# Geunwoo-Jeon/LarvaNet

Measured on AMD Instinct MI355X. Metric: HR Mpixels/s (LarvaNet x4 multi-exit train step, 48x48 LR patches), higher is better.
Workload: dtype f32; 1 GPU; LarvaNet x4 train_step_larva M4 B4,4,4,4 48ch, batch 16 of 3x48x48 -> 3x192x192 fp32 per GPU (BASELINE config 2); global_batch=16, parallelism=dp1, hip_graph=True

## Files before the change

### larvanet_amd/build.py

```python
import os
import shutil
import subprocess
import sys

CSRC = os.path.join(os.path.dirname(os.path.abspath(__file__)), "csrc")
LIB = os.path.join(CSRC, "liblarva_hip.so")
SOURCES = ["conv3x3_mfma.hip", "wgrad3x3_mfma.hip", "larva_pointwise.hip", "larva_scale.hip", "conv3x3_f16.hip",
           "larva_metrics.hip", "larva_ensemble.hip", "larva_downscale.hip", "larva_yuv.hip", "larva_resize.hip"]
HEADERS = ["larva_common.h", "larva_bicubic.h", "larva_loss.h"]
FLAGS = ["--offload-arch=gfx950", "-O3", "-std=c++17", "-fPIC", "-Wall", "-Wno-unused-function"]


def _hipcc():
    exe = shutil.which("hipcc") or "/opt/rocm/bin/hipcc"
    if not os.path.exists(exe):
        raise RuntimeError("hipcc not found: the larvanet_amd HIP library cannot be built")
    return exe


def _check_ring_waits(temps, verbose):
    import glob
    asm = glob.glob(os.path.join(temps, "conv3x3_mfma-hip-amdgcn-*.s"))
    obj = os.path.join(temps, "conv3x3_mfma.o")
    if not asm or not os.path.exists(obj):
        raise RuntimeError("larvanet_amd.build: no device assembly from the conv kernel's compile (-save-temps)")
    checker = os.path.join(os.path.dirname(os.path.dirname(CSRC)), "tools", "check_aux_loads.py")
    r = subprocess.run([sys.executable, checker, asm[0]], stdout=subprocess.PIPE, stderr=subprocess.STDOUT)
    tail = r.stdout.decode(errors="replace").strip().splitlines()[-1:]
    if verbose:
        print("[larvanet_amd.build] ring waits vs emitted loads (tools/check_aux_loads.py):", " ".join(tail), flush=True)
    if r.returncode != 0:
        sys.stderr.write(r.stdout.decode(errors="replace"))
        raise RuntimeError("larvanet_amd.build: a counted vmcnt wait of conv3x3_mfma.hip does not match the loads hipcc emitted")
    os.replace(obj, os.path.join(CSRC, "conv3x3_mfma.o"))


def _stale(target, deps):
    if not os.path.exists(target):
        return True
    t = os.path.getmtime(target)
    return any(os.path.getmtime(d) > t for d in deps)


def build_extension(force=False, verbose=True):
    import tempfile
    hipcc = _hipcc()
    hdrs = [os.path.join(CSRC, h) for h in HEADERS]
    objs = []
    procs = []
    temps = None
    for src in SOURCES:
        s = os.path.join(CSRC, src)
        o = os.path.join(CSRC, src.replace(".hip", ".o"))
        objs.append(o)
        if force or _stale(o, [s] + hdrs):
            cmd = [hipcc] + FLAGS + ["-c", s, "-o", o]
            if src == "conv3x3_mfma.hip":
                temps = tempfile.mkdtemp(prefix="build_", dir=CSRC)
                cmd = [hipcc] + FLAGS + ["-save-temps=obj", "-c", s, "-o", os.path.join(temps, "conv3x3_mfma.o")]
            if verbose:
                print("[larvanet_amd.build]", " ".join(cmd), flush=True)
            procs.append((cmd, subprocess.Popen(cmd, stdout=subprocess.PIPE, stderr=subprocess.STDOUT)))
    try:
        for cmd, p in procs:
            out, _ = p.communicate()
            if p.returncode != 0:
                sys.stderr.write(out.decode(errors="replace"))
                raise RuntimeError("hipcc failed: " + " ".join(cmd))
        if temps is not None:
            _check_ring_waits(temps, verbose)
    finally:
        if temps is not None:
            shutil.rmtree(temps, ignore_errors=True)
    if force or procs or _stale(LIB, objs):
        cmd = [hipcc, "--offload-arch=gfx950", "-shared", "-fPIC", "-o", LIB] + objs
        if verbose:
            print("[larvanet_amd.build]", " ".join(cmd), flush=True)
        subprocess.run(cmd, check=True)
    return LIB


if __name__ == "__main__":
    build_extension(force="--force" in sys.argv)
    print(LIB)
```

### larvanet_amd/csrc/conv3x3_mfma.hip

```cpp
#include "larva_common.h"
#include "larva_bicubic.h"
#include <hip/hip_ext.h>
#include <cstdlib>
#include <type_traits>

#ifndef LARVA_DIAG
#define LARVA_DIAG 0
#endif
constexpr int kWgPerCu = 2;
constexpr int kOperandDepth = 2;


#ifndef LARVA_DIAG_ONLY48
#define LARVA_DIAG_ONLY48 0
#endif

namespace larva {

#if defined(LARVA_DIAG) && (LARVA_DIAG & 32)
__device__ unsigned long long* g_stamps = nullptr;
#if LARVA_DIAG & 512
constexpr int kDiagWgPerSlot = 256;
__device__ int g_slot_of_launch = 0;
__device__ __forceinline__ void stamp_slot(unsigned long long* area, int k) {
  if (!area || threadIdx.x != 0 || blockIdx.x >= kDiagWgPerSlot) return;
  const int idx = k == 0 ? 0 : k == 2 ? 1 : k == 3 ? 2 : k == 5 ? 3
                  : !(LARVA_DIAG & 2048) ? -1 : k == 6 ? 5 : k == 7 ? 6 : k == 14 ? 7 : k == 15 ? 8 : k == 1 ? 9 : -1;
  if (idx < 0) return;
  unsigned long long* p = area + (size_t)blockIdx.x * 16;
  p[idx] = __builtin_amdgcn_s_memrealtime();
  if (k == 0) {
    const unsigned hw = __builtin_amdgcn_s_getreg((31 << 11) | 4);
    const unsigned xcc = __builtin_amdgcn_s_getreg((31 << 11) | 20);
    p[4] = (unsigned long long)hw | ((unsigned long long)xcc << 32);
  }
}
#define stamp(k) stamp_slot(a.diag_area, (k))
#else
__device__ __forceinline__ void stamp(int k) {
  if (g_stamps && threadIdx.x == 0)
    g_stamps[blockIdx.x * 16 + k] = (LARVA_DIAG & 64) ? __builtin_amdgcn_s_memtime() : __builtin_amdgcn_s_memrealtime();
}
#endif
#else
__device__ __forceinline__ void stamp(int) {}
#endif

constexpr int kCh = 8;

template <int ROWS_, int COLS_>
struct TileGeo {
  static constexpr int ROWS = ROWS_, COLS = COLS_;
  static constexpr int HALO = ROWS + 2;
  static constexpr int PC = COLS / 16;
  static constexpr int RS = COLS + 8;
  static constexpr int PS = ((HALO * RS + 15) / 32) * 32 + 16;
  static_assert(COLS % 16 == 0 && PS >= HALO * RS && PS % 32 == 16, "tile geometry");
};
using GeoWide = TileGeo<kTileRows, kTileCols>;
using GeoWide4 = TileGeo<4, kTileCols>;
using GeoS5 = TileGeo<5, 16>;
using GeoS4 = TileGeo<4, 16>;
static_assert(GeoWide::RS == kRS && GeoWide::PS == 304, "the 3 x 48 tile of larva_common.h");

struct ConvArgs {
  const float* src[kMaxSrc];
  const float* wpk;
  const float* bias;
  const float* res0;
  const float* res1;
  const float* mask;
  const float* base;
  float* out;
  int cin_per_src;
  int n_chunks;
  int N, H, W;
  int pitch;
  int tiles_x, tiles_y;
  int nwg;
  const unsigned* tile_tab;
  const float* truth;
  float* grad;
  float* partial;
  int plain_stores;
  int tab_n;
  alignas(64) int tab16[32];
  float gval;
  unsigned long long magic_tx, magic_ty, magic_cps;
#if LARVA_DIAG & 512
  unsigned long long* diag_area;
#endif
};

__host__ __device__ __forceinline__ unsigned long long div_magic(int d) { return ((1ull << 40) + d - 1) / (unsigned)d; }
__device__ __forceinline__ int div_by_magic(int n, unsigned long long magic) {
  return (int)(((unsigned long long)(unsigned)n * magic) >> 40);
}

enum Epi : int {
  kEpiPlain = 0,
  kEpiRelu = 1,
  kEpiMask = 2,
  kEpiRes1 = 3,
  kEpiRes2 = 4,
  kEpiShuffle = 5,
  kEpiShuffleBase = 6,
  kEpiShuffleL1 = 7,
  kEpiCount = 8
};

template <int COUT, typename G = GeoWide>
struct ConvCfg {
  static constexpr int CT = COUT / 16;
  static constexpr int CS = cout_stride(COUT);
  static constexpr int PS = G::PS;
  static constexpr int IN_PIECES = (kCh * PS + 255) / 256;
  static constexpr int IN_FLOATS = IN_PIECES * 256;
  static constexpr int IN_SLOTS_PER_PLANE = PS / 4;
  static constexpr int W_USED = 9 * kCh * CS;
  static constexpr int W_PIECES = (W_USED + 255) / 256;
  static constexpr int W_FLOATS = W_PIECES * 256;
  static constexpr int PIECES = IN_PIECES + W_PIECES;
  static constexpr int NPW = (PIECES + 3) / 4;
  static constexpr int STAGE_FLOATS = IN_FLOATS + W_FLOATS;
  static constexpr int STEPS = 9 * (kCh / 4);
  static constexpr int NST = 3;
  static constexpr int AHEAD = NST - 1;
  static constexpr size_t LDS_BYTES_DMA = NST * STAGE_FLOATS * sizeof(float);
  static constexpr bool LOADER = 2 * PIECES <= 63;
  static constexpr int THREADS_DMA = LOADER ? 320 : 256;
  static constexpr size_t LDS_BYTES_REG = 2 * STAGE_FLOATS * sizeof(float);
  static constexpr int RIN_SLOTS = kCh * G::HALO * (G::RS / 4);
  static constexpr int RIN_ITERS = (RIN_SLOTS + 255) / 256;
  static constexpr int RW_SLOTS = W_USED / 4;
  static constexpr int RW_ITERS = (RW_SLOTS + 255) / 256;
  static_assert(kCh * PS <= IN_FLOATS, "input planes must fit their pieces");
};

template <int COUT, typename G>
struct DmaPlan {
  unsigned voff[ConvCfg<COUT, G>::NPW];
};

template <int COUT, typename G, bool WEIGHTS>
__device__ __forceinline__ void make_plan(const ConvArgs& a, int wave, int lane, int y0, int x0,
                                          DmaPlan<COUT, G>& pl) {
  using C = ConvCfg<COUT, G>;
#pragma unroll
  for (int i = 0; i < C::NPW; ++i) {
    const int p = min(wave + 4 * i, C::PIECES - 1);
    const bool isw = p >= C::IN_PIECES;
    if constexpr (WEIGHTS) {
      if (4 * i + 3 < C::IN_PIECES) continue;
      const int ws = (p - C::IN_PIECES) * 64 + lane;
      if (isw) pl.voff[i] = (ws * 4 < C::W_USED) ? 16u * (unsigned)ws : kDmaZero;
    } else {
      if (4 * i >= C::IN_PIECES) continue;
      const int slot = p * 64 + lane;
      const int ci = slot / C::IN_SLOTS_PER_PLANE;
      const int rem = slot - ci * C::IN_SLOTS_PER_PLANE;
      const int r = rem / (G::RS / 4);
      const int q = rem - r * (G::RS / 4);
      const int gy = y0 - 1 + r, gx = x0 - 4 + 4 * q;
      const bool ok = ci < kCh && r < G::HALO && gy >= 0 && gy < a.H && gx >= 0 && gx < a.W;
      if (!isw) pl.voff[i] = ok ? 4u * (unsigned)((ci * a.H + gy) * a.pitch + gx) : kDmaZero;
    }
  }
}

struct ChunkSrc {
  i32x4 img;
  i32x4 wgt;
  const float* img_ptr;
  const float* wgt_ptr;
};

template <int COUT, typename G>
__device__ __forceinline__ ChunkSrc chunk_src(const ConvArgs& a, int chunk, int n, const float* src_override = nullptr) {
  using C = ConvCfg<COUT, G>;
  const int c0 = chunk * kCh;
  const int s_idx = div_by_magic(chunk, a.magic_cps);
  const int c_in_src = c0 - s_idx * a.cin_per_src;
  ChunkSrc cs;
  const float* src = src_override ? src_override : a.src[0];
  if (s_idx != 0) {
    asm volatile("" ::: "memory");
    src = a.src[s_idx];
  }
  cs.img_ptr = src + ((size_t)n * a.cin_per_src + c_in_src) * ((size_t)a.H * a.pitch);
  cs.wgt_ptr = a.wpk + (size_t)chunk * C::W_USED;
  cs.img = dma_rsrc(cs.img_ptr);
  cs.wgt = dma_rsrc(cs.wgt_ptr);
  return cs;
}

template <int COUT, typename G>
__device__ __forceinline__ void dma_piece(const DmaPlan<COUT, G>& pl, int i, int wave, const ChunkSrc& cs,
                                          unsigned stage_addr) {
  using C = ConvCfg<COUT, G>;
  const int p = min(wave + 4 * i, C::PIECES - 1);
  const bool isw = p >= C::IN_PIECES;
  i32x4 rsrc;
#pragma unroll
  for (int k = 0; k < 4; ++k) rsrc[k] = isw ? cs.wgt[k] : cs.img[k];
  lds_dma16_buf(rsrc, pl.voff[i], 0, stage_addr + 1024u * (unsigned)p);
}

template <int COUT, typename G>
struct LoaderPlan {
  unsigned voff[ConvCfg<COUT, G>::PIECES];
};

template <int COUT, typename G>
__device__ __forceinline__ void make_loader_plan(const ConvArgs& a, int lane, int y0, int x0, LoaderPlan<COUT, G>& pl) {
  using C = ConvCfg<COUT, G>;
#pragma unroll
  for (int p = 0; p < C::PIECES; ++p) {
    if (p < C::IN_PIECES) {
      const int slot = p * 64 + lane;
      const int ci = slot / C::IN_SLOTS_PER_PLANE;
      const int rem = slot - ci * C::IN_SLOTS_PER_PLANE;
      const int r = rem / (G::RS / 4);
      const int q = rem - r * (G::RS / 4);
      const int gy = y0 - 1 + r, gx = x0 - 4 + 4 * q;
      const bool ok = ci < kCh && r < G::HALO && gy >= 0 && gy < a.H && gx >= 0 && gx < a.W;
      pl.voff[p] = ok ? 4u * (unsigned)((ci * a.H + gy) * a.pitch + gx) : kDmaZero;
    } else {
      const int ws = (p - C::IN_PIECES) * 64 + lane;
      pl.voff[p] = (ws * 4 < C::W_USED) ? 16u * (unsigned)ws : kDmaZero;
    }
  }
}

template <int COUT, typename G>
__device__ __forceinline__ void run_loader(const ConvArgs& a, float* smem, int lane, int n, int y0, int x0) {
  using C = ConvCfg<COUT, G>;
  if constexpr ((LARVA_DIAG & 256) != 0) return;
  LoaderPlan<COUT, G> pl;
  make_loader_plan<COUT, G>(a, lane, y0, x0, pl);
  const int last = a.n_chunks - 1;
  int stage = 0;
  for (int chunk = 0; chunk <= last; ++chunk) {
    asm volatile("; LARVA_RING loader chunk_pieces=%1 ahead=%2\n\ts_waitcnt vmcnt(%0)\n\ts_barrier" ::"n"((C::AHEAD - 1) * C::PIECES), "n"(C::PIECES), "n"(C::AHEAD) : "memory");
    __builtin_amdgcn_sched_barrier(0);
    const int nstage = (stage + C::AHEAD) % C::NST;
    const unsigned dst = lds_addr_of(smem + nstage * C::STAGE_FLOATS);
    const ChunkSrc cs = chunk_src<COUT, G>(a, min(chunk + C::AHEAD, last), n);
#pragma unroll
    for (int p = 0; p < C::PIECES; ++p)
      lds_dma16_buf(p < C::IN_PIECES ? cs.img : cs.wgt, pl.voff[p], 0, dst + 1024u * (unsigned)p);
    stage = stage == C::NST - 1 ? 0 : stage + 1;
  }
  asm volatile("s_waitcnt vmcnt(0)" ::: "memory");
}

template <int COUT, typename G>
struct RegStaging {
  f32x4 in[ConvCfg<COUT, G>::RIN_ITERS];
  f32x4 w[ConvCfg<COUT, G>::RW_ITERS];
};

template <int COUT, typename G>
__device__ __forceinline__ void reg_load(const ConvArgs& a, const ChunkSrc& cs, int y0, int x0, int tid,
                                         RegStaging<COUT, G>& st) {
  using C = ConvCfg<COUT, G>;
  const size_t plane = (size_t)a.H * a.pitch;
#pragma unroll
  for (int i = 0; i < C::RIN_ITERS; ++i) {
    const int s = min(tid + i * 256, C::RIN_SLOTS - 1);
    const int ci = s / (G::HALO * (G::RS / 4));
    const int rem = s - ci * (G::HALO * (G::RS / 4));
    const int r = rem / (G::RS / 4);
    const int q = rem - r * (G::RS / 4);
    const int gy = y0 - 1 + r, gx = x0 - 4 + 4 * q;
    const bool row_ok = gy >= 0 && gy < a.H;
    const float* row = cs.img_ptr + (size_t)ci * plane + (size_t)min(max(gy, 0), a.H - 1) * a.pitch;
    f32x4 v;
#pragma unroll
    for (int e = 0; e < 4; ++e) {
      const int x = gx + e;
      const float t = row[min(max(x, 0), a.W - 1)];
      v[e] = (row_ok && x >= 0 && x < a.W) ? t : 0.f;
    }
    st.in[i] = v;
  }
#pragma unroll
  for (int i = 0; i < C::RW_ITERS; ++i) {
    const int s = min(tid + i * 256, C::RW_SLOTS - 1);
    const float* p = cs.wgt_ptr + 4 * s;
    st.w[i] = f32x4{p[0], p[1], p[2], p[3]};
  }
}

template <int COUT, typename G>
__device__ __forceinline__ void reg_store(float* stage, int tid, const RegStaging<COUT, G>& st) {
  using C = ConvCfg<COUT, G>;
#pragma unroll
  for (int i = 0; i < C::RIN_ITERS; ++i) {
    const int s = tid + i * 256;
    if (s < C::RIN_SLOTS) {
      const int ci = s / (G::HALO * (G::RS / 4));
      const int rem = s - ci * (G::HALO * (G::RS / 4));
      const int r = rem / (G::RS / 4);
      const int q = rem - r * (G::RS / 4);
      *reinterpret_cast<f32x4*>(stage + ci * C::PS + r * G::RS + 4 * q) = st.in[i];
    }
  }
#pragma unroll
  for (int i = 0; i < C::RW_ITERS; ++i) {
    const int s = tid + i * 256;
    if (s < C::RW_SLOTS) *reinterpret_cast<f32x4*>(stage + C::IN_FLOATS + 4 * s) = st.w[i];
  }
}

template <int COUT, typename G, int NCT, int PG0, int NPG>
__device__ __forceinline__ void read_operands(const float* const (&a_base)[NCT], const float* b_base, int step,
                                              float (&av)[NCT], float (&bv)[NPG]) {
  using C = ConvCfg<COUT, G>;
  if constexpr ((LARVA_DIAG & 128) != 0) {
#pragma unroll
    for (int c = 0; c < NCT; ++c) av[c] = (float)step;
#pragma unroll
    for (int p = 0; p < NPG; ++p) bv[p] = (float)(step + p);
    return;
  }
  const int tap = step / (kCh / 4), kk = step % (kCh / 4);
  const int ky = tap / 3, kx = tap % 3;
#pragma unroll
  for (int c = 0; c < NCT; ++c) av[c] = a_base[c][(tap * kCh + kk * 4) * C::CS];
#pragma unroll
  for (int p = 0; p < NPG; ++p) {
    const int pg = PG0 + p, prow = pg / G::PC, pcol = pg % G::PC;
    bv[p] = b_base[kk * 4 * C::PS + (prow + ky) * G::RS + pcol * 16 + kx];
  }
}

template <int NMF, int NRD, int M>
__device__ __forceinline__ void shadow_groups() {
  if constexpr (M < NMF) {
    __builtin_amdgcn_sched_group_barrier(0x8, 1, 0);
    constexpr int share = (NRD + NMF - 1 - M) / NMF;
    if constexpr (share > 0) __builtin_amdgcn_sched_group_barrier(0x100, share, 0);
    shadow_groups<NMF, NRD, M + 1>();
  }
}

template <int COUT, typename G, int NCT, int PG0, int NPG, bool SWAP>
__device__ __forceinline__ void mfma_chunk(const float* stage, int ct0, int lane, f32x4 (&acc)[NCT][NPG],
                                           const float* wstage = nullptr) {
  using C = ConvCfg<COUT, G>;
  const int lr = lane & 15, lq = lane >> 4;
  const float* const wrows = wstage ? wstage : stage + C::IN_FLOATS;
  const float* a_base[NCT];
#pragma unroll
  for (int c = 0; c < NCT; ++c)
    a_base[c] = wrows + lq * C::CS + lr + (cout_swizzled(COUT) ? (((ct0 + c) ^ (lq & 1)) * 16) : (ct0 + c) * 16);
  const float* b_base = stage + lq * C::PS + lr + 3;
  constexpr int D = kOperandDepth;
  float av[D + 1][NCT], bv[D + 1][NPG];
#pragma unroll
  for (int d = 0; d < D; ++d)
    if (d < C::STEPS) read_operands<COUT, G, NCT, PG0, NPG>(a_base, b_base, d, av[d], bv[d]);
#pragma unroll
  for (int step = 0; step < C::STEPS; ++step) {
    __builtin_amdgcn_sched_barrier(0);
    if (step + D < C::STEPS)
      read_operands<COUT, G, NCT, PG0, NPG>(a_base, b_base, step + D, av[(step + D) % (D + 1)], bv[(step + D) % (D + 1)]);
    constexpr int NMF = NCT * NPG;
    constexpr int NRD = NCT + NPG;
#pragma unroll
    for (int m = 0; m < NMF; ++m) {
      const float wv = av[step % (D + 1)][m / NPG], xv = bv[step % (D + 1)][m % NPG];
      acc[m / NPG][m % NPG] = __builtin_amdgcn_mfma_f32_16x16x4f32(SWAP ? xv : wv, SWAP ? wv : xv, acc[m / NPG][m % NPG], 0, 0, 0);
    }
    shadow_groups<NMF, NRD, 0>();
    __builtin_amdgcn_sched_barrier(0);
  }
}

template <int KEEP, int PIECES, int AUX>
__device__ __forceinline__ void wait_and_barrier() {
  static_assert(KEEP == PIECES + AUX, "a ring wait keeps exactly the next chunk's pieces and the operand loads in flight");
  asm volatile("; LARVA_RING pieces=%1 aux=%2\n\ts_waitcnt vmcnt(%0)\n\ts_barrier" ::"n"(KEEP), "n"(PIECES), "n"(AUX) : "memory");
  __builtin_amdgcn_sched_barrier(0);
}

template <typename G>
__device__ __forceinline__ void decode_tile(const ConvArgs& a, int vb, int& n, int& y0, int& x0) {
  const int tile = xcd_remap(vb, a.nwg);
  const int t2 = div_by_magic(tile, a.magic_tx);
  const int tx = tile - t2 * a.tiles_x;
  n = div_by_magic(t2, a.magic_ty);
  const int ty = t2 - n * a.tiles_y;
  x0 = tx * G::COLS;
  y0 = ty * G::ROWS;
}

template <int COUT, typename G, bool VEC, int EPI, int NCT, int PG0, int NPG, bool PERSIST = false>
__device__ __forceinline__ void run_role(const ConvArgs& a, float* smem, int ct0, int wave, int n, int y0, int x0, int tid) {
  using C = ConvCfg<COUT, G>;
  static_assert(!VEC || C::LOADER, "the 16-byte path runs with a loader wave (2 * PIECES <= 63 for every instantiated shape)");
  static_assert(!PERSIST || VEC, "persistent tiles: the loader-wave path");
  const int lane = tid & 63;
  const int lr = lane & 15, lq = lane >> 4;
  float* const out_ptr = a.out;
  struct { int H, W, pitch, plain; } k = {a.H, a.W, a.pitch, a.plain_stores};
  asm volatile("" : "+s"(k.H), "+s"(k.W), "+s"(k.pitch), "+s"(k.plain));

  constexpr bool kShuffleEpi = (EPI == kEpiShuffle || EPI == kEpiShuffleBase || EPI == kEpiShuffleL1);
  constexpr bool kPixMajor = VEC && !kShuffleEpi;
  f32x4 bias[NCT];
#pragma unroll
  for (int c = 0; c < NCT; ++c) bias[c] = f32x4{0.f, 0.f, 0.f, 0.f};
  auto load_bias = [&]() {
    if (a.bias) {
#pragma unroll
      for (int c = 0; c < NCT; ++c)
#pragma unroll
        for (int r = 0; r < 4; ++r) bias[c][r] = a.bias[(ct0 + c) * 16 + (kPixMajor ? lr : lq * 4 + r)];
    }
  };

  constexpr int NAUX = (EPI == kEpiMask || EPI == kEpiRes1 || EPI == kEpiShuffleBase)
                           ? 1 : ((EPI == kEpiRes2 || EPI == kEpiShuffleL1) ? 2 : 0);
  f32x4 aux[NAUX > 0 ? NAUX : 1][NAUX > 0 ? NCT : 1][NAUX > 0 ? NPG : 1];
  constexpr int NU = NCT * NPG;
  constexpr int kEarlyPairs = PERSIST && COUT == 48 ? (NAUX * NU < 7 ? NAUX * NU : 7) : NAUX * NU;
  constexpr int kLatePart = 4, kEarlyAll = 5;
  auto load_aux = [&](int part = -1) {
#pragma unroll
    for (int c = 0; c < NCT; ++c)
#pragma unroll
      for (int p = 0; p < NPG; ++p) {
        const int pg = PG0 + p, prow = pg / G::PC, pcol = pg % G::PC;
        const int y = min(y0 + prow, a.H - 1), x = min(x0 + pcol * 16 + lr, a.W - 1);
        auto want = [&](int op) {
          const int q = op * NU + c * NPG + p;
          return part < 0 ? true : part == kLatePart ? q >= kEarlyPairs : q < kEarlyPairs;
        };
        if constexpr (kShuffleEpi) {
          const int HH = 4 * a.H, WW = 4 * a.W;
          const size_t idx = (((size_t)n * C::CT + (ct0 + c)) * HH + (4 * y + lq)) * WW + 4 * x;
          if (want(0)) aux[0][c][p] = *reinterpret_cast<const f32x4*>(a.base + idx);
          if constexpr (EPI == kEpiShuffleL1) {
            if (want(1)) aux[1][c][p] = *reinterpret_cast<const f32x4*>(a.truth + idx);
          }
        } else if constexpr (kPixMajor && (PERSIST || G::COLS == 16)) {
          const unsigned plane = (unsigned)a.H * (unsigned)a.pitch;
          const unsigned lane_off = 4u * ((unsigned)lr * plane + (unsigned)lq * 4u);
          const int soff = __builtin_amdgcn_readfirstlane(
              (int)(4u * ((unsigned)((ct0 + c) * 16) * plane + (unsigned)(y0 + prow) * (unsigned)a.pitch + (unsigned)(x0 + pcol * 16))));
          auto image = [&](const float* t) {
            const unsigned long long b = reinterpret_cast<unsigned long long>(t + (size_t)n * COUT * plane);
            const unsigned lo = (unsigned)__builtin_amdgcn_readfirstlane((int)(unsigned)b);
            const unsigned hi = (unsigned)__builtin_amdgcn_readfirstlane((int)(unsigned)(b >> 32));
            return __builtin_amdgcn_make_buffer_rsrc(reinterpret_cast<void*>(((unsigned long long)hi << 32) | lo), 0,
                                                     (int)(COUT * plane * 4u), 0x00020000);
          };
          if constexpr (EPI == kEpiMask) {
            if (want(0)) aux[0][c][p] = __builtin_bit_cast(f32x4, __builtin_amdgcn_raw_buffer_load_b128(image(a.mask), lane_off, soff, 0));
          }
          if constexpr (EPI == kEpiRes1 || EPI == kEpiRes2) {
            if (want(0)) aux[0][c][p] = __builtin_bit_cast(f32x4, __builtin_amdgcn_raw_buffer_load_b128(image(a.res0), lane_off, soff, 0));
          }
          if constexpr (EPI == kEpiRes2) {
            if (want(1)) aux[1][c][p] = __builtin_bit_cast(f32x4, __builtin_amdgcn_raw_buffer_load_b128(image(a.res1), lane_off, soff, 0));
          }
        } else if constexpr (kPixMajor) {
          const size_t plane = (size_t)a.H * a.pitch;
          const int xb = min(x0 + pcol * 16 + lq * 4, a.pitch - 4);
          const size_t idx = ((size_t)n * COUT + (ct0 + c) * 16 + lr) * plane + (size_t)y * a.pitch + xb;
          if constexpr (EPI == kEpiMask) {
            if (want(0)) aux[0][c][p] = *reinterpret_cast<const f32x4*>(a.mask + idx);
          }
          if constexpr (EPI == kEpiRes1 || EPI == kEpiRes2) {
            if (want(0)) aux[0][c][p] = *reinterpret_cast<const f32x4*>(a.res0 + idx);
          }
          if constexpr (EPI == kEpiRes2) {
            if (want(1)) aux[1][c][p] = *reinterpret_cast<const f32x4*>(a.res1 + idx);
          }
        } else {
          const size_t plane = (size_t)a.H * a.pitch;
          const size_t idx0 = ((size_t)n * COUT + (ct0 + c) * 16 + lq * 4) * plane + (size_t)y * a.pitch + x;
#pragma unroll
          for (int r = 0; r < 4; ++r) {
            if constexpr (EPI == kEpiMask) aux[0][c][p][r] = a.mask[idx0 + r * plane];
            if constexpr (EPI == kEpiRes1 || EPI == kEpiRes2) aux[0][c][p][r] = a.res0[idx0 + r * plane];
            if constexpr (EPI == kEpiRes2) aux[1][c][p][r] = a.res1[idx0 + r * plane];
          }
        }
      }
  };
  constexpr bool kAuxLate = VEC && !kShuffleEpi && !(LARVA_DIAG & 6) && NAUX > 0 && !PERSIST;
  constexpr int kAuxLoads = kAuxLate ? NAUX * NCT * NPG : 0;
  auto load_early = [&]() {
    load_bias();
    if constexpr (NAUX > 0 && !kAuxLate && !(LARVA_DIAG & 4)) load_aux();
  };
  int pstage = 0;
  for (int vb = blockIdx.x;; vb += gridDim.x) {
  if constexpr (PERSIST) {
    if (vb >= a.nwg) break;
    decode_tile<G>(a, vb, n, y0, x0);
  }
  if constexpr (!VEC || (LARVA_DIAG & 2)) load_early();

  f32x4 acc[NCT][NPG];
#pragma unroll
  for (int c = 0; c < NCT; ++c)
#pragma unroll
    for (int p = 0; p < NPG; ++p) acc[c][p] = f32x4{0.f, 0.f, 0.f, 0.f};

  if constexpr (PERSIST) {
    load_bias();
    const int my_chunk = a.n_chunks >= 4 ? (wave & 3) : 0;
    __builtin_amdgcn_sched_barrier(0);
    for (int chunk = 0; chunk < a.n_chunks; ++chunk) {
      asm volatile("s_barrier" ::: "memory");
      __builtin_amdgcn_sched_barrier(0);
      if constexpr (NAUX > 0) {
        if (chunk == my_chunk) load_aux(kEarlyAll);
        __builtin_amdgcn_sched_barrier(0);
      }
      mfma_chunk<COUT, G, NCT, PG0, NPG, kPixMajor>(smem + pstage * C::STAGE_FLOATS, ct0, lane, acc);
      pstage = pstage == C::NST - 1 ? 0 : pstage + 1;
    }
    asm volatile("s_waitcnt vmcnt(0)" ::: "memory");
    __builtin_amdgcn_sched_barrier(0);
    if constexpr (kEarlyPairs < NAUX * NU) {
      load_aux(kLatePart);
      __builtin_amdgcn_sched_barrier(0);
    }
  } else if constexpr (VEC) {
    DmaPlan<COUT, G> pl;
    const int last = a.n_chunks - 1;
    if constexpr (!(LARVA_DIAG & 2)) {
      const ChunkSrc cs0 = chunk_src<COUT, G>(a, 0, n);
      const unsigned st0 = lds_addr_of(smem), st1 = lds_addr_of(smem + C::STAGE_FLOATS);
      stamp(6);
      make_plan<COUT, G, true>(a, wave, lane, y0, x0, pl);
#pragma unroll
      for (int i = 0; i < C::NPW; ++i)
        if (wave + 4 * i >= C::IN_PIECES) dma_piece<COUT, G>(pl, i, wave, cs0, st0);
      __builtin_amdgcn_sched_barrier(0);
      stamp(7);
      load_early();
      stamp(14);
      make_plan<COUT, G, false>(a, wave, lane, y0, x0, pl);
#pragma unroll
      for (int i = 0; i < C::NPW; ++i)
        if (wave + 4 * i < C::IN_PIECES) dma_piece<COUT, G>(pl, i, wave, cs0, st0);
      stamp(15);
      const ChunkSrc cs1 = chunk_src<COUT, G>(a, min(1, last), n);
#pragma unroll
      for (int i = 0; i < C::NPW; ++i) dma_piece<COUT, G>(pl, i, wave, cs1, st1);
      if constexpr (kAuxLate) {
        __builtin_amdgcn_sched_barrier(0);
        load_aux();
        __builtin_amdgcn_sched_barrier(0);
      }
    }
    stamp(1);
    int stage = 0;
    for (int chunk = 0; chunk <= last; ++chunk) {
      if constexpr ((LARVA_DIAG & 256) != 0) {
      } else if (chunk == 0) wait_and_barrier<((LARVA_DIAG & 2) ? 0 : C::NPW) + kAuxLoads, ((LARVA_DIAG & 2) ? 0 : C::NPW), kAuxLoads>();
      else wait_and_barrier<kAuxLoads, 0, kAuxLoads>();
      if (chunk == 0) stamp(2);
      stamp(8 + (chunk < 7 ? chunk : 7));
      if constexpr (!(LARVA_DIAG & 1)) mfma_chunk<COUT, G, NCT, PG0, NPG, kPixMajor>(smem + stage * C::STAGE_FLOATS, ct0, lane, acc);
      stage = stage == C::NST - 1 ? 0 : stage + 1;
    }
    asm volatile("s_waitcnt vmcnt(0)" ::: "memory");
    stamp(3);
  } else {
    RegStaging<COUT, G> st;
    if constexpr (!(LARVA_DIAG & 2)) {
      reg_load<COUT, G>(a, chunk_src<COUT, G>(a, 0, n), y0, x0, tid, st);
      reg_store<COUT, G>(smem, tid, st);
    }
    __syncthreads();
    for (int chunk = 0; chunk < a.n_chunks; ++chunk) {
      float* cur = smem + (chunk & 1) * C::STAGE_FLOATS;
      float* nxt = smem + ((chunk & 1) ^ 1) * C::STAGE_FLOATS;
      const bool more = chunk + 1 < a.n_chunks;
      if constexpr (!(LARVA_DIAG & 2)) {
        if (more) reg_load<COUT, G>(a, chunk_src<COUT, G>(a, chunk + 1, n), y0, x0, tid, st);
      }
      if constexpr (!(LARVA_DIAG & 1)) mfma_chunk<COUT, G, NCT, PG0, NPG, kPixMajor>(cur, ct0, lane, acc);
      if constexpr (!(LARVA_DIAG & 2)) {
        if (more) reg_store<COUT, G>(nxt, tid, st);
      }
      __syncthreads();
    }
  }

  if constexpr ((LARVA_DIAG & 4) != 0) {
#pragma unroll
    for (int c = 0; c < NCT; ++c)
#pragma unroll
      for (int p = 0; p < NPG; ++p) asm volatile("" ::"v"(acc[c][p]));
    return;
  }

  if constexpr (EPI == kEpiShuffleL1) {
    const int HH = 4 * k.H, WW = 4 * k.W;
    const size_t plane = (size_t)k.H * k.pitch;
    const float g = a.gval;
    float s = 0.f;
#pragma unroll
    for (int c = 0; c < NCT; ++c)
#pragma unroll
      for (int p = 0; p < NPG; ++p) {
        const int pg = PG0 + p, prow = pg / G::PC, pcol = pg % G::PC;
        const int y = y0 + prow, x = x0 + pcol * 16 + lr;
        const f32x4 v = (acc[c][p] + bias[c]) + aux[0][c][p];
        if (y < k.H && x < k.W) {
          if (out_ptr) {
            const size_t idx = (((size_t)n * C::CT + (ct0 + c)) * HH + (4 * y + lq)) * WW + 4 * x;
            __builtin_nontemporal_store(v, reinterpret_cast<f32x4*>(out_ptr + idx));
          }
          const f32x4 d = v - aux[1][c][p];
          s += fabsf(d[0]) + fabsf(d[1]) + fabsf(d[2]) + fabsf(d[3]);
          const size_t idx0 = ((size_t)n * COUT + (ct0 + c) * 16 + lq * 4) * plane + (size_t)y * k.pitch + x;
#pragma unroll
          for (int r = 0; r < 4; ++r)
            __builtin_nontemporal_store(d[r] > 0.f ? g : (d[r] < 0.f ? -g : 0.f), &a.grad[idx0 + r * plane]);
        }
      }
#pragma unroll
    for (int o = 32; o > 0; o >>= 1) s += __shfl_xor(s, o);
    if (lane == 0) a.partial[4 * blockIdx.x + wave] = s;
  } else if constexpr (EPI == kEpiShuffle || EPI == kEpiShuffleBase) {
    const int HH = 4 * k.H, WW = 4 * k.W;
#pragma unroll
    for (int c = 0; c < NCT; ++c)
#pragma unroll
      for (int p = 0; p < NPG; ++p) {
        const int pg = PG0 + p, prow = pg / G::PC, pcol = pg % G::PC;
        const int y = y0 + prow, x = x0 + pcol * 16 + lr;
        const size_t idx = (((size_t)n * C::CT + (ct0 + c)) * HH + (4 * y + lq)) * WW + 4 * x;
        f32x4 v = acc[c][p] + bias[c];
        if constexpr (EPI == kEpiShuffleBase) v += aux[0][c][p];
        if (y < k.H && x < k.W) __builtin_nontemporal_store(v, reinterpret_cast<f32x4*>(out_ptr + idx));
      }
  } else if constexpr (kPixMajor) {
    const size_t plane = (size_t)k.H * k.pitch;
    auto store_all = [&](auto plain_tag, auto interior_tag) {
      constexpr bool kPlain = decltype(plain_tag)::value;
      constexpr bool kInterior = decltype(interior_tag)::value;
#pragma unroll
      for (int c = 0; c < NCT; ++c)
#pragma unroll
        for (int p = 0; p < NPG; ++p) {
          const int pg = PG0 + p, prow = pg / G::PC, pcol = pg % G::PC;
          const int y = y0 + prow, xb = x0 + pcol * 16 + lq * 4;
          const size_t idx = ((size_t)n * COUT + (ct0 + c) * 16 + lr) * plane + (size_t)y * k.pitch + xb;
          f32x4 v = acc[c][p] + bias[c];
          if (kInterior || (y < k.H && xb < k.pitch)) {
#pragma unroll
            for (int r = 0; r < 4; ++r) {
              float o = v[r];
              if constexpr (EPI == kEpiRelu) o = fmaxf(o, 0.f);
              if constexpr (EPI == kEpiMask) o = (aux[0][c][p][r] > 0.f) ? o : 0.f;
              if constexpr (EPI == kEpiRes1 || EPI == kEpiRes2) o += aux[0][c][p][r];
              if constexpr (EPI == kEpiRes2) o += aux[1][c][p][r];
              v[r] = (kInterior || xb + r < k.W) ? o : 0.f;
            }
            if constexpr (kPlain) *reinterpret_cast<f32x4*>(out_ptr + idx) = v;
            else __builtin_nontemporal_store(v, reinterpret_cast<f32x4*>(out_ptr + idx));
          }
        }
    };
    constexpr bool kFastPath = EPI == kEpiPlain || EPI == kEpiRelu || EPI == kEpiRes1;
    const bool interior = kFastPath && y0 + G::ROWS <= k.H && x0 + G::COLS <= k.W;
    auto store_policy = [&](auto plain_tag) {
      if constexpr (kFastPath) {
        if (interior) {
          store_all(plain_tag, std::true_type{});
          return;
        }
      }
      store_all(plain_tag, std::false_type{});
    };
    if constexpr ((LARVA_DIAG & 16) != 0) {
      store_policy(std::true_type{});
    } else if constexpr (G::COLS == 16) {
      if (k.plain) store_policy(std::true_type{});
      else store_policy(std::false_type{});
    } else {
      store_policy(std::false_type{});
    }
  } else {
    const size_t plane = (size_t)k.H * k.pitch;
#pragma unroll
    for (int c = 0; c < NCT; ++c)
#pragma unroll
      for (int p = 0; p < NPG; ++p) {
        const int pg = PG0 + p, prow = pg / G::PC, pcol = pg % G::PC;
        const int y = y0 + prow, x = x0 + pcol * 16 + lr;
        const size_t idx0 = ((size_t)n * COUT + (ct0 + c) * 16 + lq * 4) * plane + (size_t)y * k.pitch + x;
        const f32x4 v = acc[c][p] + bias[c];
        if (y < k.H && x < k.pitch) {
          const bool real = x < k.W;
#pragma unroll
          for (int r = 0; r < 4; ++r) {
            float o = v[r];
            if constexpr (EPI == kEpiRelu) o = fmaxf(o, 0.f);
            if constexpr (EPI == kEpiMask) o = (aux[0][c][p][r] > 0.f) ? o : 0.f;
            if constexpr (EPI == kEpiRes1 || EPI == kEpiRes2) o += aux[0][c][p][r];
            if constexpr (EPI == kEpiRes2) o += aux[1][c][p][r];
            o = real ? o : 0.f;
            if constexpr ((LARVA_DIAG & 16) != 0) out_ptr[idx0 + r * plane] = o;
            else __builtin_nontemporal_store(o, &out_ptr[idx0 + r * plane]);
          }
        }
      }
  }
#if LARVA_DIAG & 32
  stamp(4);
  asm volatile("s_waitcnt vmcnt(0)" ::: "memory");
  stamp(5);
#endif
  if constexpr (!PERSIST) break;
  }
}

__device__ __forceinline__ void fetch_args(const ConvArgs& a) {
  asm volatile("" ::"s"(a.src[0]), "s"(a.wpk), "s"(a.bias), "s"(a.out), "s"(a.cin_per_src), "s"(a.n_chunks), "s"(a.N),
               "s"(a.H), "s"(a.W), "s"(a.pitch), "s"(a.tiles_x), "s"(a.tiles_y), "s"(a.magic_tx), "s"(a.magic_ty),
               "s"(a.magic_cps), "s"(a.nwg), "s"(a.tile_tab), "s"(a.plain_stores), "s"(a.tab_n),
               "s"(a.tab16[0]), "s"(a.tab16[16]));
}

template <int COUT, bool VEC, int EPI, typename G = GeoWide>
__device__ __forceinline__ void conv_tile(const ConvArgs& a, float* smem) {
  if constexpr ((LARVA_DIAG & 8) != 0) return;
  stamp(0);
  fetch_args(a);
  const int tile = xcd_remap(blockIdx.x, a.nwg);
  const int t2 = div_by_magic(tile, a.magic_tx);
  const int tx = tile - t2 * a.tiles_x;
  const int n = div_by_magic(t2, a.magic_ty);
  const int ty = t2 - n * a.tiles_y;
  const int x0 = tx * G::COLS, y0 = ty * G::ROWS;
  const int tid = threadIdx.x;
  const int wave = __builtin_amdgcn_readfirstlane(tid >> 6);
  __builtin_amdgcn_s_setprio(1);

  if constexpr (VEC) {
    if (wave == 4) {
      if constexpr (!(LARVA_DIAG & 2)) run_loader<COUT, G>(a, smem, tid & 63, n, y0, x0);
      return;
    }
  }
  if constexpr (G::ROWS == 4) {
    static_assert(VEC && (COUT == 48 || COUT == 32), "4 x 48 tiles: the 16-byte path at 48 / 32 channels");
    if constexpr (COUT == 48) {
      if (wave < 3) run_role<COUT, G, VEC, EPI, 1, 0, 9>(a, smem, wave, wave, n, y0, x0, tid);
      else run_role<COUT, G, VEC, EPI, 3, 9, 3>(a, smem, 0, wave, n, y0, x0, tid);
    } else {
      if (wave < 2) run_role<COUT, G, VEC, EPI, 1, 0, 6>(a, smem, wave, wave, n, y0, x0, tid);
      else run_role<COUT, G, VEC, EPI, 1, 6, 6>(a, smem, wave - 2, wave, n, y0, x0, tid);
    }
  } else if constexpr (COUT == 48) {
    if (wave < 3) run_role<COUT, G, VEC, EPI, 1, 0, 7>(a, smem, wave, wave, n, y0, x0, tid);
    else run_role<COUT, G, VEC, EPI, 3, 7, 2>(a, smem, 0, wave, n, y0, x0, tid);
  } else if constexpr (COUT == 32) {
    if (wave < 2) run_role<COUT, G, VEC, EPI, 1, 0, 5>(a, smem, wave, wave, n, y0, x0, tid);
    else run_role<COUT, G, VEC, EPI, 1, 5, 4>(a, smem, wave - 2, wave, n, y0, x0, tid);
  } else {
    static_assert(COUT == 64, "unsupported channel count");
    run_role<COUT, G, VEC, EPI, 1, 0, 9>(a, smem, wave, wave, n, y0, x0, tid);
  }
}

template <int COUT, bool VEC, int EPI>
__global__ __launch_bounds__(VEC ? ConvCfg<COUT>::THREADS_DMA : 256, VEC ? kWgPerCu : 1) void conv3x3_mfma_kernel(ConvArgs a) {
  extern __shared__ __attribute__((aligned(16))) float smem[];
  conv_tile<COUT, VEC, EPI>(a, smem);
}

template <int COUT, int EPI>
__global__ __launch_bounds__((ConvCfg<COUT, GeoWide4>::THREADS_DMA), kWgPerCu) void conv3x3_mfma_rows4_kernel(ConvArgs a) {
  extern __shared__ __attribute__((aligned(16))) float smem[];
  conv_tile<COUT, true, EPI, GeoWide4>(a, smem);
}
static_assert(2 * ConvCfg<48, GeoWide4>::LDS_BYTES_DMA <= 160 * 1024, "two 4 x 48 workgroups per CU");

template <int COUT, typename G>
__device__ __forceinline__ void run_loader_persist(const ConvArgs& a, float* smem, int lane) {
  using C = ConvCfg<COUT, G>;
  static_assert(C::NST == 3 && 2 * C::PIECES <= 63, "three stages, two chunks in flight");
  LoaderPlan<COUT, G> pl;
  int vb_i = blockIdx.x, n_i, y0, x0, c_i = 0, s_i = 0;
  decode_tile<G>(a, vb_i, n_i, y0, x0);
  make_loader_plan<COUT, G>(a, lane, y0, x0, pl);
  bool more = true;
  auto issue = [&]() {
    const ChunkSrc cs = chunk_src<COUT, G>(a, c_i, n_i);
    const unsigned dst = lds_addr_of(smem + s_i * C::STAGE_FLOATS);
#pragma unroll
    for (int p = 0; p < C::PIECES; ++p)
      lds_dma16_buf(p < C::IN_PIECES ? cs.img : cs.wgt, pl.voff[p], 0, dst + 1024u * (unsigned)p);
    s_i = s_i == C::NST - 1 ? 0 : s_i + 1;
    if (++c_i == a.n_chunks) {
      c_i = 0;
      vb_i += gridDim.x;
      more = vb_i < a.nwg;
      if (more) {
        decode_tile<G>(a, vb_i, n_i, y0, x0);
        make_loader_plan<COUT, G>(a, lane, y0, x0, pl);
      }
    }
  };
  int ahead = 0;
  issue();
  ++ahead;
  if (more) {
    issue();
    ++ahead;
  }
  while (ahead > 0) {
    if (ahead == 2) asm volatile("s_waitcnt vmcnt(%0)" ::"n"(C::PIECES) : "memory");
    else asm volatile("s_waitcnt vmcnt(0)" ::: "memory");
    asm volatile("s_barrier" ::: "memory");
    __builtin_amdgcn_sched_barrier(0);
    --ahead;
    if (more) {
      issue();
      ++ahead;
    }
  }
}

template <int COUT, int EPI>
__global__ __launch_bounds__((ConvCfg<COUT>::THREADS_DMA), kWgPerCu) void conv3x3_mfma_persist_kernel(ConvArgs a) {
  extern __shared__ __attribute__((aligned(16))) float smem[];
  using G = GeoWide;
  stamp(0);
  fetch_args(a);
  const int tid = threadIdx.x;
  const int wave = __builtin_amdgcn_readfirstlane(tid >> 6);
  __builtin_amdgcn_s_setprio(1);
  if (wave == 4) {
    run_loader_persist<COUT, G>(a, smem, tid & 63);
    return;
  }
  if constexpr (COUT == 48) {
    if (wave < 3) run_role<COUT, G, true, EPI, 1, 0, 7, true>(a, smem, wave, wave, 0, 0, 0, tid);
    else run_role<COUT, G, true, EPI, 3, 7, 2, true>(a, smem, 0, wave, 0, 0, 0, tid);
  } else if constexpr (COUT == 32) {
    if (wave < 2) run_role<COUT, G, true, EPI, 1, 0, 5, true>(a, smem, wave, wave, 0, 0, 0, tid);
    else run_role<COUT, G, true, EPI, 1, 5, 4, true>(a, smem, wave - 2, wave, 0, 0, 0, tid);
  } else {
    static_assert(COUT == 64, "unsupported channel count");
    run_role<COUT, G, true, EPI, 1, 0, 9, true>(a, smem, wave, wave, 0, 0, 0, tid);
  }
}

template <int COUT, int EPI, typename G>
__device__ __forceinline__ void strip_roles(const ConvArgs& a, float* smem, int wave, int n, int y0, int x0, int tid) {
  static_assert(ConvCfg<COUT, G>::LOADER, "the strip kernel is launched with a loader wave");
  static_assert(COUT == 48 || COUT == 32 || COUT == 64, "strip tiles: 32, 48 or 64 output channels");
  if (wave == 4) {
    run_loader<COUT, G>(a, smem, tid & 63, n, y0, x0);
    return;
  }
  if constexpr (COUT == 64) {
    run_role<COUT, G, true, EPI, 1, 0, G::ROWS>(a, smem, wave, wave, n, y0, x0, tid);
  } else if constexpr (COUT == 48) {
    if (wave < 3) run_role<COUT, G, true, EPI, 1, 0, G::ROWS - 1>(a, smem, wave, wave, n, y0, x0, tid);
    else run_role<COUT, G, true, EPI, 3, G::ROWS - 1, 1>(a, smem, 0, wave, n, y0, x0, tid);
  } else if constexpr (G::ROWS == 5) {
    if (wave < 2) run_role<COUT, G, true, EPI, 1, 0, 3>(a, smem, wave, wave, n, y0, x0, tid);
    else if (wave == 2) run_role<COUT, G, true, EPI, 2, 3, 1>(a, smem, 0, wave, n, y0, x0, tid);
    else run_role<COUT, G, true, EPI, 2, 4, 1>(a, smem, 0, wave, n, y0, x0, tid);
  } else {
    if (wave < 2) run_role<COUT, G, true, EPI, 1, 0, 2>(a, smem, wave, wave, n, y0, x0, tid);
    else run_role<COUT, G, true, EPI, 1, 2, 2>(a, smem, wave - 2, wave, n, y0, x0, tid);
  }
}

template <int COUT, int EPI>
__global__ __launch_bounds__(320, kWgPerCu) void conv3x3_mfma_strip_kernel(ConvArgs a) {
  extern __shared__ __attribute__((aligned(16))) float smem[];
  stamp(0);
  fetch_args(a);
  const int tile = xcd_remap(blockIdx.x, a.nwg);
  const int n = div_by_magic(tile, a.magic_tx);
  const int slot = tile - n * a.tiles_x;
  unsigned e;
  if (a.tab_n) {
    const unsigned pair = (unsigned)a.tab16[slot >> 1];
    const unsigned h = (slot & 1) ? pair >> 16 : pair & 0xffffu;
    e = (h & 0xffu) | (((h >> 8) & 0x7fu) << 16) | ((h >> 15) << 31);
  } else {
    e = a.tile_tab[slot];
  }
  const int y0 = (int)(e & 0xfffu), x0 = (int)((e >> 12) & 0xfffu);
  const int tid = threadIdx.x;
  const int wave = __builtin_amdgcn_readfirstlane(tid >> 6);
  __builtin_amdgcn_s_setprio(1);
  if (e >> 31) strip_roles<COUT, EPI, GeoS5>(a, smem, wave, n, y0, x0, tid);
  else strip_roles<COUT, EPI, GeoS4>(a, smem, wave, n, y0, x0, tid);
}
template <int COUT>
constexpr size_t kStripLdsBytes = ConvCfg<COUT, GeoS5>::LDS_BYTES_DMA > ConvCfg<COUT, GeoS4>::LDS_BYTES_DMA ? ConvCfg<COUT, GeoS5>::LDS_BYTES_DMA
                                                                                                            : ConvCfg<COUT, GeoS4>::LDS_BYTES_DMA;
static_assert(kWgPerCu * kStripLdsBytes<48> <= 160 * 1024 && kWgPerCu * kStripLdsBytes<64> <= 160 * 1024, "strip workgroups per CU");

constexpr int kMaxConvJobs = 4;
struct ConvBatch {
  ConvArgs job[kMaxConvJobs];
};

template <int COUT, int EPI>
__global__ __launch_bounds__(ConvCfg<COUT>::THREADS_DMA, kWgPerCu) void conv3x3_mfma_batch_kernel(ConvBatch b) {
  extern __shared__ __attribute__((aligned(16))) float smem[];
  conv_tile<COUT, true, EPI>(b.job[blockIdx.y], smem);
}

constexpr int kMaxPackJobs = 64;

struct PackJob {
  const float* w;
  float* fwd;
  float* bwd;
  int cout, cin, w_cin_total, w_cin_off;
};

struct PackBatch {
  PackJob job[kMaxPackJobs];
};

__host__ __device__ constexpr int packed_floats(int cout, int cin) {
  return (cin / kCh) * 9 * kCh * cout_stride(cout);
}

constexpr int kPackTileCols = 64;
constexpr int kPackLd = kPackTileCols + 1;
constexpr int kPackTileFloats = 9 * kCh * kPackLd;

__host__ __device__ constexpr int pack_slots(int cout, int cin) { return cin / kCh + cout / kCh; }

__device__ __forceinline__ void pack_block(const PackJob& j, int slot, float* __restrict__ tile) {
  const int nfc = j.cin / kCh;
  const bool fwd = slot < nfc;
  const int chunk = fwd ? slot : slot - nfc;
  float* __restrict__ out = fwd ? j.fwd : j.bwd;
  if ((!fwd && chunk >= j.cout / kCh) || !out) return;
  const int cols = fwd ? j.cout : j.cin;
  const int cs = cout_stride(cols);
  const int tid = threadIdx.x;
  out += (size_t)chunk * 72 * cs;
  for (int c0 = 0; c0 < cs; c0 += kPackTileCols) {
    const int ncol = min(kPackTileCols, cols - c0);
    if (fwd) {
      for (int idx = tid; idx < ncol * 72; idx += 256) {
        const int c = idx / 72, r = idx - c * 72, k = r / 9, tap = r - k * 9;
        const int cin_abs = j.w_cin_off + chunk * kCh + k;
        tile[(tap * kCh + k) * kPackLd + c] =
            cin_abs < j.w_cin_total ? j.w[((size_t)(c0 + c) * j.w_cin_total + cin_abs) * 9 + tap] : 0.f;
      }
    } else {
      const int row = ncol * 9;
      for (int idx = tid; idx < kCh * row; idx += 256) {
        const int k = idx / row, rem = idx - k * row, c = rem / 9, tap = rem - c * 9;
        tile[((8 - tap) * kCh + k) * kPackLd + c] =
            j.w_cin_off + c0 + c < j.w_cin_total
                ? j.w[((size_t)(chunk * kCh + k) * j.w_cin_total + j.w_cin_off + c0) * 9 + rem] : 0.f;
      }
    }
    __syncthreads();
    const int wcols = min(kPackTileCols, cs - c0);
    const bool swz = cout_swizzled(cols);
    for (int idx = tid; idx < 72 * wcols; idx += 256) {
      const int r = idx / wcols, c = idx - r * wcols;
      const int col = swz ? ((c0 + c) ^ ((r & 1) << 4)) : c0 + c;
      out[r * cs + col] = c < ncol ? tile[r * kPackLd + c] : 0.f;
    }
    __syncthreads();
  }
}

__global__ __launch_bounds__(256) void pack_weights_batch_kernel(PackBatch b) {
  __shared__ float tile[kPackTileFloats];
  pack_block(b.job[blockIdx.y], blockIdx.x, tile);
}

constexpr int kPrologueBlocks = 192;
constexpr int kProloguePadSlices = 2, kPrologueBicSlices = 8;
struct PrologueArgs {
  PackBatch packs;
  int npack, slots;
  const float* x;
  float* x16;
  float* base;
  int N, C, H, W;
};

__global__ __launch_bounds__(256) void step_prologue_kernel(PrologueArgs a) {
  __shared__ float tile[kPackTileFloats];
  int blk = blockIdx.x;
  if (blk < a.npack * a.slots) {
    const int job = blk / a.slots;
    pack_block(a.packs.job[job], blk - job * a.slots, tile);
    return;
  }
  blk -= a.npack * a.slots;
  constexpr int nthr = kPrologueBlocks * 256;
  const int slice = blk / kPrologueBlocks, tid = (blk - slice * kPrologueBlocks) * 256 + threadIdx.x;
  const int nbic = a.base ? kPrologueBicSlices : 0;
  if (slice < nbic) {
    bicubic4_body(a.x, a.base, a.N * a.C, a.H, a.W, (long long)slice * nthr + tid, (long long)nthr * kPrologueBicSlices);
  } else {
    const int plane = a.H * a.W, per_img = a.C * plane, total = a.N * per_img;
    for (int i = (slice - nbic) * nthr + tid; i < total; i += nthr * kProloguePadSlices) {
      const int n = i / per_img, r = i - n * per_img;
      a.x16[(size_t)n * 16 * plane + r] = a.x[i];
    }
  }
}

struct LaunchTiming {
  hipEvent_t start, stop;
};

template <auto Kernel, typename Args>
static hipError_t launch(dim3 grid, dim3 block, size_t lds, hipStream_t stream, const LaunchTiming* tm, const Args& a) {
  static PerDeviceOnce lds_set;
  if (const hipError_t e = ensure_dynamic_lds(lds_set, reinterpret_cast<const void*>(Kernel), lds); e != hipSuccess) return e;
  if (tm)
    hipExtLaunchKernelGGL(Kernel, grid, block, lds, stream, tm->start, tm->stop, 0, a);
  else
    hipLaunchKernelGGL(Kernel, grid, block, lds, stream, a);
  return hipGetLastError();
}

template <int... E>
struct EpiSet {
  static constexpr bool has(int epi) { return ((epi == E) || ...); }
};
using EpiAll = EpiSet<kEpiPlain, kEpiRelu, kEpiMask, kEpiRes1, kEpiRes2, kEpiShuffle, kEpiShuffleBase>;
using EpiBatch48 = EpiSet<kEpiPlain, kEpiRelu, kEpiMask, kEpiRes1, kEpiRes2, kEpiShuffle, kEpiShuffleBase, kEpiShuffleL1>;
using EpiInference = EpiSet<kEpiPlain, kEpiRelu, kEpiRes1, kEpiRes2, kEpiShuffle, kEpiShuffleBase>;
using EpiRows4 = EpiInference;
using EpiPersist = EpiInference;

template <int... E, typename F>
static hipError_t with_epi(EpiSet<E...>, int epi, hipError_t absent, F&& f) {
  hipError_t r = absent;
  (void)((epi == E && (r = f(std::integral_constant<int, E>{}), true)) || ...);
  return r;
}

template <typename F>
static hipError_t with_cout(int cout, hipError_t absent, F&& f) {
  switch (cout) {
#if !LARVA_DIAG_ONLY48
    case 32: return f(std::integral_constant<int, 32>{});
    case 64: return f(std::integral_constant<int, 64>{});
#endif
    case 48: return f(std::integral_constant<int, 48>{});
    default: return absent;
  }
}

static int conv_slots() { return kWgPerCu * device_cu_count(); }

template <int COUT>
static hipError_t launch_conv(const ConvArgs& a, bool vec, int epi, hipStream_t stream, const LaunchTiming* tm) {
  using C = ConvCfg<COUT>;
  const dim3 grid(a.N * a.tiles_x * a.tiles_y);
  return with_epi(EpiAll{}, epi, hipErrorInvalidValue, [&](auto e) {
    constexpr int EPI = decltype(e)::value;
    if (vec)
      return launch<conv3x3_mfma_kernel<COUT, true, EPI>>(grid, dim3(C::THREADS_DMA), C::LDS_BYTES_DMA, stream, tm, a);
    return launch<conv3x3_mfma_kernel<COUT, false, EPI>>(grid, dim3(256), C::LDS_BYTES_REG, stream, tm, a);
  });
}

template <int COUT>
static hipError_t launch_rows4(const ConvArgs& a, int epi, hipStream_t stream, const LaunchTiming* tm) {
  using C = ConvCfg<COUT, GeoWide4>;
  return with_epi(EpiRows4{}, epi, hipErrorNotSupported, [&](auto e) {
    return launch<conv3x3_mfma_rows4_kernel<COUT, decltype(e)::value>>(dim3(a.nwg), dim3(C::THREADS_DMA), C::LDS_BYTES_DMA,
                                                                      stream, tm, a);
  });
}

template <int COUT>
static hipError_t launch_persist(const ConvArgs& a, int epi, hipStream_t stream, const LaunchTiming* tm) {
  using C = ConvCfg<COUT>;
  if ((long long)COUT * a.H * a.pitch * 4 >= (1ll << 31)) return hipErrorNotSupported;
  const int grid = a.nwg < conv_slots() ? a.nwg : conv_slots();
  return with_epi(EpiPersist{}, epi, hipErrorNotSupported, [&](auto e) {
    return launch<conv3x3_mfma_persist_kernel<COUT, decltype(e)::value>>(dim3(grid), dim3(C::THREADS_DMA), C::LDS_BYTES_DMA,
                                                                        stream, tm, a);
  });
}

template <int COUT>
static hipError_t launch_batch(const ConvBatch& b, int njobs, int epi, hipStream_t stream) {
  using C = ConvCfg<COUT>;
  using Set = std::conditional_t<COUT == 48, EpiBatch48, EpiAll>;
  const ConvArgs& a = b.job[0];
  return with_epi(Set{}, epi, epi == kEpiShuffleL1 ? hipErrorNotSupported : hipErrorInvalidValue, [&](auto e) {
    return launch<conv3x3_mfma_batch_kernel<COUT, decltype(e)::value>>(dim3(a.N * a.tiles_x * a.tiles_y, njobs),
                                                                      dim3(C::THREADS_DMA), C::LDS_BYTES_DMA, stream,
                                                                      nullptr, b);
  });
}

template <int COUT>
static hipError_t launch_strip(const ConvArgs& a, int epi, hipStream_t stream, const LaunchTiming* tm) {
  return with_epi(EpiAll{}, epi, hipErrorInvalidValue, [&](auto e) {
    return launch<conv3x3_mfma_strip_kernel<COUT, decltype(e)::value>>(dim3(a.nwg), dim3(320), kStripLdsBytes<COUT>, stream,
                                                                      tm, a);
  });
}

}

using namespace larva;

extern "C" {

long long larva_packed_weight_floats(int cout, int cin) { return (long long)packed_floats(cout, cin); }

static int fill_pack_jobs(PackBatch& b, const float* const* w, float* const* wpk_fwd, float* const* wpk_bwd,
                          const int* cout, const int* cin, const int* w_cin_total, const int* w_cin_off, int njobs) {
  int slots = 0;
  for (int i = 0; i < njobs; ++i) {
    if (!w[i] || cout[i] % kCh || cin[i] % kCh || cout[i] <= 0 || cin[i] <= 0) return -1;
    b.job[i] = PackJob{w[i], wpk_fwd[i], wpk_bwd[i], cout[i], cin[i], w_cin_total[i], w_cin_off[i]};
    const int n = pack_slots(cout[i], cin[i]);
    slots = n > slots ? n : slots;
  }
  return slots;
}

int larva_pack_weights_batch(const float* const* w, float* const* wpk_fwd, float* const* wpk_bwd,
                             const int* cout, const int* cin, const int* w_cin_total,
                             const int* w_cin_off, int njobs, void* stream) {
  if (njobs < 1 || njobs > kMaxPackJobs) return (int)hipErrorInvalidValue;
  PackBatch b{};
  const int slots = fill_pack_jobs(b, w, wpk_fwd, wpk_bwd, cout, cin, w_cin_total, w_cin_off, njobs);
  if (slots < 1) return (int)hipErrorInvalidValue;
  hipLaunchKernelGGL(pack_weights_batch_kernel, dim3(slots, njobs), dim3(256), 0, (hipStream_t)stream, b);
  return (int)hipGetLastError();
}

int larva_step_prologue(const float* const* w, float* const* wpk_fwd, float* const* wpk_bwd, const int* cout,
                        const int* cin, const int* w_cin_total, const int* w_cin_off, int njobs, const float* x,
                        float* x16, float* base, int N, int C, int H, int W, void* stream) {
  if (njobs < 0 || njobs > kMaxPackJobs || !x || N <= 0 || C <= 0 || C > 16 || H <= 0 || W <= 0)
    return (int)hipErrorInvalidValue;
  if ((long long)N * 16 * H * W >= (1ll << 31)) return (int)hipErrorInvalidValue;
  if (base && (reinterpret_cast<uintptr_t>(base) & 15)) return (int)hipErrorInvalidValue;
  PrologueArgs a{};
  a.slots = njobs ? fill_pack_jobs(a.packs, w, wpk_fwd, wpk_bwd, cout, cin, w_cin_total, w_cin_off, njobs) : 0;
  if (a.slots < 0) return (int)hipErrorInvalidValue;
  a.npack = njobs;
  a.x = x; a.x16 = x16; a.base = base;
  a.N = N; a.C = C; a.H = H; a.W = W;
  if (!x16 && base) return (int)hipErrorInvalidValue;
  const int blocks = njobs * a.slots + kPrologueBlocks * ((base ? kPrologueBicSlices : 0) + (x16 ? kProloguePadSlices : 0));
  if (blocks == 0) return 0;
  hipLaunchKernelGGL(step_prologue_kernel, dim3(blocks), dim3(256), 0, (hipStream_t)stream, a);
  return (int)hipGetLastError();
}

int larva_pack_weights(const float* w, float* wpk_fwd, float* wpk_bwd, int cout, int cin,
                       int w_cin_total, int w_cin_off, void* stream) {
  return larva_pack_weights_batch(&w, &wpk_fwd, &wpk_bwd, &cout, &cin, &w_cin_total, &w_cin_off, 1, stream);
}

#if LARVA_DIAG & 512
static int g_diag_next_slot = -1, g_diag_slot_cap = 0;
static unsigned long long* g_diag_host_base = nullptr;
static int diag_take_slot() {
  if (g_diag_next_slot < 0 || g_diag_next_slot >= g_diag_slot_cap) return -1;
  return g_diag_next_slot++;
}
int larva_diag_arm_slots(int first, int cap) {
  const int was = g_diag_next_slot;
  g_diag_next_slot = first;
  g_diag_slot_cap = cap;
  return was;
}
int larva_diag_next_slot(void) { return g_diag_next_slot; }
#endif

static int conv_build(const float* const* src, int n_src, int cin_per_src, const float* wpk, const float* bias,
                      const float* res0, const float* res1, const float* mask, const float* base, float* out,
                      int N, int H, int W, int pitch, int relu, int mode, ConvArgs& a, bool& aligned, int& epi) {
  if (pitch == 0) pitch = W;
  if (pitch < W) return (int)hipErrorInvalidValue;
  if (n_src < 1 || n_src > kMaxSrc || cin_per_src % kCh || cin_per_src <= 0 || N <= 0 || H <= 0 || W <= 0)
    return (int)hipErrorInvalidValue;
  if (mode != 0 && mode != 1) return (int)hipErrorInvalidValue;
  if ((long long)cin_per_src * H * pitch >= (1ll << 31)) return (int)hipErrorInvalidValue;
  if (!wpk || !out) return (int)hipErrorInvalidValue;
  a = ConvArgs{};
#if LARVA_DIAG & 512
  {
    const int slot = diag_take_slot();
    a.diag_area = (slot >= 0 && g_diag_host_base) ? g_diag_host_base + (size_t)slot * kDiagWgPerSlot * 16 : nullptr;
  }
#endif
  aligned = (pitch % 4 == 0) && ((reinterpret_cast<uintptr_t>(wpk) & 15) == 0);
  for (int i = 0; i < n_src; ++i) {
    if (!src[i]) return (int)hipErrorInvalidValue;
    a.src[i] = src[i];
    aligned = aligned && ((reinterpret_cast<uintptr_t>(src[i]) & 15) == 0);
  }
  aligned = aligned && (((reinterpret_cast<uintptr_t>(out) | reinterpret_cast<uintptr_t>(res0) |
                          reinterpret_cast<uintptr_t>(res1) | reinterpret_cast<uintptr_t>(mask)) & 15) == 0);
  a.wpk = wpk; a.bias = bias; a.res0 = res0; a.res1 = res1; a.mask = mask; a.base = base;
  a.out = out;
  a.cin_per_src = cin_per_src;
  a.n_chunks = n_src * cin_per_src / kCh;
  a.N = N; a.H = H; a.W = W; a.pitch = pitch;
  a.tiles_x = (pitch + kTileCols - 1) / kTileCols;
  a.tiles_y = (H + kTileRows - 1) / kTileRows;
  if ((long long)N * a.tiles_x * a.tiles_y >= (1ll << 20)) return (int)hipErrorInvalidValue;
  a.magic_tx = div_magic(a.tiles_x);
  a.magic_ty = div_magic(a.tiles_y);
  a.magic_cps = div_magic(cin_per_src / kCh);
  a.nwg = N * a.tiles_x * a.tiles_y;
  if (mode == 1) {
    if (relu || mask || res0 || res1) return (int)hipErrorInvalidValue;
    epi = base ? kEpiShuffleBase : kEpiShuffle;
  } else {
    if (base) return (int)hipErrorInvalidValue;
    const int code = (relu ? 1 : 0) | (mask ? 2 : 0) | (res0 ? 4 : 0) | (res1 ? 8 : 0);
    switch (code) {
      case 0: epi = kEpiPlain; break;
      case 1: epi = kEpiRelu; break;
      case 2: epi = kEpiMask; break;
      case 4: epi = kEpiRes1; break;
      case 12: epi = kEpiRes2; break;
      default: return (int)hipErrorInvalidValue;
    }
  }
  return 0;
}

static int conv_tile_rows(int N, int H, int pitch, int cout, int epi, bool aligned, int forced) {
  const bool can4 = aligned && (cout == 48 || cout == 32) && EpiRows4::has(epi);
  if (forced == 3 || !can4) return 3;
  if (forced == 4) return 4;
  const long long tiles3 = (long long)N * ((pitch + kTileCols - 1) / kTileCols) * ((H + 2) / 3);
  return (cout == 32 && tiles3 > conv_slots()) ? 4 : 3;
}

static int conv_dispatch(const float* const* src, int n_src, int cin_per_src, const float* wpk,
                         const float* bias, const float* res0, const float* res1, const float* mask,
                         const float* base, float* out, int N, int cout, int H, int W, int pitch, int relu,
                         int mode, void* stream, const LaunchTiming* tm, int tile_rows = 0) {
  ConvArgs a;
  bool aligned;
  int epi;
  const int rc = conv_build(src, n_src, cin_per_src, wpk, bias, res0, res1, mask, base, out, N, H, W, pitch, relu,
                            mode, a, aligned, epi);
  if (rc) return rc;
  hipStream_t s = (hipStream_t)stream;
  if (tile_rows != 0 && tile_rows != 3 && tile_rows != 4) return (int)hipErrorInvalidValue;
  if (conv_tile_rows(N, H, a.pitch, cout, epi, aligned, tile_rows) == 4) {
    a.tiles_y = (H + 3) / 4;
    a.magic_ty = div_magic(a.tiles_y);
    a.nwg = N * a.tiles_x * a.tiles_y;
    return (int)with_cout(cout, hipErrorInvalidValue, [&](auto c) {
      if constexpr (decltype(c)::value == 64) return hipErrorNotSupported;
      else return launch_rows4<decltype(c)::value>(a, epi, s, tm);
    });
  }
  if (tile_rows == 4) return (int)hipErrorNotSupported;
  const char* pe = getenv("LARVA_PERSIST");
  const bool persist_on = !(pe && pe[0] == '0');
  if (persist_on && aligned && a.nwg > conv_slots()) {
    const hipError_t e = with_cout(cout, hipErrorNotSupported, [&](auto c) {
      return launch_persist<decltype(c)::value>(a, epi, s, tm);
    });
    if (e != hipErrorNotSupported) return (int)e;
  }
  return (int)with_cout(cout, hipErrorInvalidValue, [&](auto c) {
    return launch_conv<decltype(c)::value>(a, aligned, epi, s, tm);
  });
}

int larva_conv3x3_fwd(const float* const* src, int n_src, int cin_per_src, const float* wpk,
                      const float* bias, const float* res0, const float* res1, const float* mask,
                      const float* base, float* out, int N, int cout, int H, int W, int relu,
                      int mode, void* stream) {
  return conv_dispatch(src, n_src, cin_per_src, wpk, bias, res0, res1, mask, base, out, N, cout, H, W, 0, relu,
                       mode, stream, nullptr);
}

int larva_conv3x3_fwd_pitched(const float* const* src, int n_src, int cin_per_src, const float* wpk,
                              const float* bias, const float* res0, const float* res1, const float* mask,
                              const float* base, float* out, int N, int cout, int H, int W, int pitch,
                              int relu, int mode, void* stream) {
  return conv_dispatch(src, n_src, cin_per_src, wpk, bias, res0, res1, mask, base, out, N, cout, H, W, pitch,
                       relu, mode, stream, nullptr);
}

int larva_conv3x3_fwd_tiled(const float* const* src, int n_src, int cin_per_src, const float* wpk,
                            const float* bias, const float* res0, const float* res1, const float* mask,
                            const float* base, float* out, int N, int cout, int H, int W, int pitch,
                            int relu, int mode, int tile_rows, void* stream) {
  return conv_dispatch(src, n_src, cin_per_src, wpk, bias, res0, res1, mask, base, out, N, cout, H, W, pitch,
                       relu, mode, stream, nullptr, tile_rows);
}

int larva_conv3x3_fwd_batch(int njobs, const float* const* src, int n_src, int cin_per_src,
                            const float* const* wpk, const float* const* bias, const float* const* res0,
                            const float* const* res1, const float* const* mask, const float* const* base,
                            float* const* out, int N, int cout, int H, int W, int pitch, int relu, int mode,
                            void* stream) {
  if (njobs < 2 || njobs > kMaxConvJobs || !src || !wpk || !out) return (int)hipErrorInvalidValue;
  ConvBatch b{};
  int epi0 = -1;
  for (int j = 0; j < njobs; ++j) {
    bool aligned;
    int epi;
    const int rc = conv_build(src + (size_t)j * n_src, n_src, cin_per_src, wpk[j], bias ? bias[j] : nullptr,
                              res0 ? res0[j] : nullptr, res1 ? res1[j] : nullptr, mask ? mask[j] : nullptr,
                              base ? base[j] : nullptr, out[j], N, H, W, pitch, relu, mode, b.job[j], aligned, epi);
    if (rc) return rc;
    if (!aligned) return (int)hipErrorNotSupported;
    if (j > 0 && epi != epi0) return (int)hipErrorInvalidValue;
    epi0 = epi;
  }
  return (int)with_cout(cout, hipErrorInvalidValue, [&](auto c) {
    return launch_batch<decltype(c)::value>(b, njobs, epi0, (hipStream_t)stream);
  });
}

int larva_exit_l1_partials(int N, int H, int pitch) {
  return 4 * N * ((pitch + kTileCols - 1) / kTileCols) * ((H + kTileRows - 1) / kTileRows);
}

int larva_conv3x3_exit_l1_batch(int njobs, const float* const* src, int n_src, int cin_per_src,
                                const float* const* wpk, const float* const* bias, const float* const* base,
                                const float* const* truth, float* const* out, float* const* grad,
                                float* const* partial, float gval, int N, int cout, int H, int W, int pitch,
                                void* stream) {
  if (njobs < 2 || njobs > kMaxConvJobs || !src || !wpk || !base || !truth || !out || !grad || !partial)
    return (int)hipErrorInvalidValue;
  if (cout != 48) return (int)hipErrorNotSupported;
  ConvBatch b{};
  for (int j = 0; j < njobs; ++j) {
    bool aligned;
    int epi;
    if (!base[j] || !truth[j] || !grad[j] || !partial[j]) return (int)hipErrorInvalidValue;
    const int rc = conv_build(src + (size_t)j * n_src, n_src, cin_per_src, wpk[j], bias ? bias[j] : nullptr, nullptr,
                              nullptr, nullptr, base[j], grad[j], N, H, W, pitch, 0, 1, b.job[j], aligned, epi);
    if (rc) return rc;
    if (!aligned || ((reinterpret_cast<uintptr_t>(truth[j]) | reinterpret_cast<uintptr_t>(base[j])) & 15))
      return (int)hipErrorNotSupported;
    b.job[j].out = out[j];
    b.job[j].truth = truth[j];
    b.job[j].grad = grad[j];
    b.job[j].partial = partial[j];
    b.job[j].gval = gval;
  }
  return (int)launch_batch<48>(b, njobs, kEpiShuffleL1, (hipStream_t)stream);
}

int larva_strip_tile_table(int H, int W, int phase, unsigned* tab, int cap) {
  if (H <= 0 || W <= 0 || H >= 4096 || W >= 4096 || !tab || cap < 0) return -1;
  int n5 = 0, n4 = 0;
  for (int pass = 0; pass < 2; ++pass) {
    int fives = 0, fours = 0, i5 = 0, i4 = 0;
    for (int x0 = 0; x0 < W; x0 += 16) {
      int best_a = -1, best_gap = 1 << 30;
      for (int a5 = 0; 5 * a5 <= H; ++a5) {
        if ((H - 5 * a5) % 4) continue;
        const int b4 = (H - 5 * a5) / 4;
        const int gap = (fives + a5) - (fours + b4);
        const int g = gap < 0 ? -gap : gap;
        if (g < best_gap) { best_gap = g; best_a = a5; }
      }
      if (best_a < 0) return -2;
      const int a5 = best_a, b4 = (H - 5 * a5) / 4;
      fives += a5; fours += b4;
      if (pass == 0) continue;
      int y = 0, ra = a5, rb = b4;
      while (ra > 0 || rb > 0) {
        const bool five = ra > 0 && (rb == 0 || (long long)ra * b4 >= (long long)rb * a5);
        const int k = five ? i5++ : i4++;
        const int mine = five ? n5 : n4, other = five ? n4 : n5;
        const bool first = five == (phase == 0);
        int slot;
        if (k < other) slot = 2 * k + (first ? 0 : 1);
        else slot = 2 * other + (k - other);
        (void)mine;
        if (slot < cap) tab[slot] = (unsigned)y | ((unsigned)x0 << 12) | (five ? 0x80000000u : 0u);
        y += five ? 5 : 4;
        if (five) --ra; else --rb;
      }
    }
    n5 = fives; n4 = fours;
  }
  return n5 + n4;
}

static int strips_dispatch(const float* const* src, int n_src, int cin_per_src, const float* wpk,
                           const float* bias, const float* res0, const float* res1, const float* mask,
                           const float* base, float* out, int N, int cout, int H, int W, int pitch,
                           int relu, int mode, const unsigned* tile_tab, const unsigned* tile_tab_host,
                           int tiles_per_image, int plain_stores, void* stream, const LaunchTiming* tm) {
  if (cout != 48 && cout != 32 && cout != 64) return (int)hipErrorNotSupported;
  if (!tile_tab || tiles_per_image < 1) return (int)hipErrorInvalidValue;
  ConvArgs a;
  bool aligned;
  int epi;
  const int rc = conv_build(src, n_src, cin_per_src, wpk, bias, res0, res1, mask, base, out, N, H, W, pitch, relu,
                            mode, a, aligned, epi);
  if (rc) return rc;
  if (!aligned) return (int)hipErrorNotSupported;
  if ((long long)N * tiles_per_image >= (1ll << 20)) return (int)hipErrorInvalidValue;
  if ((long long)cout * H * a.pitch * 4 >= (1ll << 31)) return (int)hipErrorNotSupported;
  a.tile_tab = tile_tab;
  if (tile_tab_host && tiles_per_image <= 64 && H <= 256 && pitch <= 2048) {
    a.tab_n = tiles_per_image;
    for (int t = 0; t < tiles_per_image; ++t) {
      const unsigned e = tile_tab_host[t];
      const unsigned y0 = e & 0xfffu, x0 = (e >> 12) & 0xfffu;
      if (y0 > 255u || (x0 & 15u) || (x0 >> 4) > 127u) { a.tab_n = 0; break; }
      const unsigned h = y0 | ((x0 >> 4) << 8) | ((e >> 31) << 15);
      a.tab16[t >> 1] |= (int)(h << ((t & 1) * 16));
    }
  }
  a.plain_stores = plain_stores ? 1 : 0;
  a.tiles_x = tiles_per_image;
  a.tiles_y = 1;
  a.magic_tx = div_magic(tiles_per_image);
  a.magic_ty = div_magic(1);
  a.nwg = N * tiles_per_image;
  return (int)with_cout(cout, hipErrorNotSupported, [&](auto c) {
    return launch_strip<decltype(c)::value>(a, epi, (hipStream_t)stream, tm);
  });
}

int larva_conv3x3_fwd_strips(const float* const* src, int n_src, int cin_per_src, const float* wpk,
                             const float* bias, const float* res0, const float* res1, const float* mask,
                             const float* base, float* out, int N, int cout, int H, int W, int pitch,
                             int relu, int mode, const unsigned* tile_tab, const unsigned* tile_tab_host,
                             int tiles_per_image, int plain_stores, void* stream) {
  return strips_dispatch(src, n_src, cin_per_src, wpk, bias, res0, res1, mask, base, out, N, cout, H, W, pitch, relu, mode,
                         tile_tab, tile_tab_host, tiles_per_image, plain_stores, stream, nullptr);
}

#if LARVA_DIAG & 32
int larva_diag_set_stamps(unsigned long long* buf) {
#if LARVA_DIAG & 512
  g_diag_host_base = buf;
#endif
  return (int)hipMemcpyToSymbol(HIP_SYMBOL(larva::g_stamps), &buf, sizeof(buf));
}
#endif

}
```

Before: 366.0 HR Mpixels/s.

## Preload leading conv kernel arguments into SGPRs and prefetch strip weights early

Conv kernels now take their hot scalar parameters (weight/source pointers, tile magics, sizes) as leading scalar arguments, and the build passes an LLVM flag so that the first kernarg dwords are preloaded into SGPRs. The goal is to remove the kernarg-load latency at the start of each short conv workgroup. The strip kernel also issues the weight DMA before decoding its tile, with WPRE skipping the later weight load and GeoS4 padded to match GeoS5's piece count. A build check enforces that preload is present and that VGPRs stay within 128, which adds build fragility and more register pressure.

Result: slower. 361.9 HR Mpixels/s (-1.1%).

```diff
diff --git a/larvanet_amd/build.py b/larvanet_amd/build.py
--- a/larvanet_amd/build.py
+++ b/larvanet_amd/build.py
@@ -9,6 +9,8 @@
            "larva_metrics.hip", "larva_ensemble.hip", "larva_downscale.hip", "larva_yuv.hip", "larva_resize.hip"]
 HEADERS = ["larva_common.h", "larva_bicubic.h", "larva_loss.h"]
 FLAGS = ["--offload-arch=gfx950", "-O3", "-std=c++17", "-fPIC", "-Wall", "-Wno-unused-function"]
+KERNARG_PRELOAD_DWORDS = 14
+CONV_FLAGS = ["-mllvm", "-amdgpu-kernarg-preload-count=%d" % KERNARG_PRELOAD_DWORDS]
 
 
 def _hipcc():
@@ -35,6 +37,35 @@
     os.replace(obj, os.path.join(CSRC, "conv3x3_mfma.o"))
 
 
+def _check_preload(temps, verbose):
+    import glob
+    import re
+    asm = glob.glob(os.path.join(temps, "conv3x3_mfma-hip-amdgcn-*.s"))
+    text = open(asm[0]).read()
+    kernels = re.findall(r"\.amdhsa_kernel (_ZN5larva\d+conv3x3_mfma_\w*kernel\w+)(.*?)\.end_amdhsa_kernel", text, re.S)
+    if not kernels:
+        raise RuntimeError("larvanet_amd.build: no conv3x3_mfma_*_kernel descriptors in the device assembly")
+
+    def field(body, name):
+        m = re.search(r"\.amdhsa_%s (\d+)" % name, body)
+        return int(m.group(1)) if m else 0
+
+    missing = [n for n, b in kernels if field(b, "user_sgpr_kernarg_preload_length") == 0]
+    if missing:
+        raise RuntimeError("larvanet_amd.build: conv kernels without kernarg preload (leading scalar parameters and "
+                           "CONV_FLAGS): " + ", ".join(missing[:4]))
+    train = [(n, b) for n, b in kernels if re.search(r"conv3x3_mfma_(strip|batch)_kernelILi48E", n)]
+    over = [(n, field(b, "next_free_vgpr")) for n, b in train if field(b, "next_free_vgpr") > 128]
+    if over:
+        raise RuntimeError("larvanet_amd.build: more than 128 VGPRs (two workgroups per CU): %s" % over)
+    if verbose:
+        print("[larvanet_amd.build] %d conv kernels, preload %s dwords, user SGPRs %s; training-path instances: max %d VGPRs, "
+              "max %d SGPRs" % (len(kernels), sorted({field(b, "user_sgpr_kernarg_preload_length") for _, b in kernels}),
+                                sorted({field(b, "user_sgpr_count") for _, b in kernels}),
+                                max(field(b, "next_free_vgpr") for _, b in train),
+                                max(field(b, "next_free_sgpr") for _, b in train)), flush=True)
+
+
 def _stale(target, deps):
     if not os.path.exists(target):
         return True
@@ -57,7 +88,7 @@
             cmd = [hipcc] + FLAGS + ["-c", s, "-o", o]
             if src == "conv3x3_mfma.hip":
                 temps = tempfile.mkdtemp(prefix="build_", dir=CSRC)
-                cmd = [hipcc] + FLAGS + ["-save-temps=obj", "-c", s, "-o", os.path.join(temps, "conv3x3_mfma.o")]
+                cmd = [hipcc] + FLAGS + CONV_FLAGS + ["-save-temps=obj", "-c", s, "-o", os.path.join(temps, "conv3x3_mfma.o")]
             if verbose:
                 print("[larvanet_amd.build]", " ".join(cmd), flush=True)
             procs.append((cmd, subprocess.Popen(cmd, stdout=subprocess.PIPE, stderr=subprocess.STDOUT)))
@@ -68,6 +99,7 @@
                 sys.stderr.write(out.decode(errors="replace"))
                 raise RuntimeError("hipcc failed: " + " ".join(cmd))
         if temps is not None:
+            _check_preload(temps, verbose)
             _check_ring_waits(temps, verbose)
     finally:
         if temps is not None:
diff --git a/larvanet_amd/csrc/conv3x3_mfma.hip b/larvanet_amd/csrc/conv3x3_mfma.hip
--- a/larvanet_amd/csrc/conv3x3_mfma.hip
+++ b/larvanet_amd/csrc/conv3x3_mfma.hip
@@ -35,7 +35,7 @@
     p[4] = (unsigned long long)hw | ((unsigned long long)xcc << 32);
   }
 }
-#define stamp(k) stamp_slot(a.diag_area, (k))
+#define stamp(slot_) stamp_slot(a.k.diag_area, (slot_))
 #else
 __device__ __forceinline__ void stamp(int k) {
   if (g_stamps && threadIdx.x == 0)
@@ -48,9 +48,9 @@
 
 constexpr int kCh = 8;
 
-template <int ROWS_, int COLS_>
+template <int ROWS_, int COLS_, int MIN_IN_PIECES_ = 0>
 struct TileGeo {
-  static constexpr int ROWS = ROWS_, COLS = COLS_;
+  static constexpr int ROWS = ROWS_, COLS = COLS_, MIN_IN_PIECES = MIN_IN_PIECES_;
   static constexpr int HALO = ROWS + 2;
   static constexpr int PC = COLS / 16;
   static constexpr int RS = COLS + 8;
@@ -60,7 +60,7 @@
 using GeoWide = TileGeo<kTileRows, kTileCols>;
 using GeoWide4 = TileGeo<4, kTileCols>;
 using GeoS5 = TileGeo<5, 16>;
-using GeoS4 = TileGeo<4, 16>;
+using GeoS4 = TileGeo<4, 16, 6>;
 static_assert(GeoWide::RS == kRS && GeoWide::PS == 304, "the 3 x 48 tile of larva_common.h");
 
 struct ConvArgs {
@@ -92,6 +92,20 @@
 #endif
 };
 
+struct ConvView {
+  const float* wpk;
+  const float* src0;
+  const float* bias;
+  int H, W, pitch, cin_per_src, n_chunks;
+  int nwg, tiles_x, tiles_y;
+  unsigned long long magic_tx, magic_ty, magic_cps;
+  const ConvArgs& k;
+};
+__device__ __forceinline__ ConvView view_of(const ConvArgs& k) {
+  return ConvView{k.wpk, k.src[0], k.bias, k.H, k.W, k.pitch, k.cin_per_src, k.n_chunks, k.nwg, k.tiles_x, k.tiles_y,
+                  k.magic_tx, k.magic_ty, k.magic_cps, k};
+}
+
 __host__ __device__ __forceinline__ unsigned long long div_magic(int d) { return ((1ull << 40) + d - 1) / (unsigned)d; }
 __device__ __forceinline__ int div_by_magic(int n, unsigned long long magic) {
   return (int)(((unsigned long long)(unsigned)n * magic) >> 40);
@@ -114,7 +128,7 @@
   static constexpr int CT = COUT / 16;
   static constexpr int CS = cout_stride(COUT);
   static constexpr int PS = G::PS;
-  static constexpr int IN_PIECES = (kCh * PS + 255) / 256;
+  static constexpr int IN_PIECES = (kCh * PS + 255) / 256 > G::MIN_IN_PIECES ? (kCh * PS + 255) / 256 : G::MIN_IN_PIECES;
   static constexpr int IN_FLOATS = IN_PIECES * 256;
   static constexpr int IN_SLOTS_PER_PLANE = PS / 4;
   static constexpr int W_USED = 9 * kCh * CS;
@@ -143,7 +157,7 @@
 };
 
 template <int COUT, typename G, bool WEIGHTS>
-__device__ __forceinline__ void make_plan(const ConvArgs& a, int wave, int lane, int y0, int x0,
+__device__ __forceinline__ void make_plan(const ConvView& a, int wave, int lane, int y0, int x0,
                                           DmaPlan<COUT, G>& pl) {
   using C = ConvCfg<COUT, G>;
 #pragma unroll
@@ -176,16 +190,16 @@
 };
 
 template <int COUT, typename G>
-__device__ __forceinline__ ChunkSrc chunk_src(const ConvArgs& a, int chunk, int n, const float* src_override = nullptr) {
+__device__ __forceinline__ ChunkSrc chunk_src(const ConvView& a, int chunk, int n, const float* src_override = nullptr) {
   using C = ConvCfg<COUT, G>;
   const int c0 = chunk * kCh;
   const int s_idx = div_by_magic(chunk, a.magic_cps);
   const int c_in_src = c0 - s_idx * a.cin_per_src;
   ChunkSrc cs;
-  const float* src = src_override ? src_override : a.src[0];
+  const float* src = src_override ? src_override : a.src0;
   if (s_idx != 0) {
     asm volatile("" ::: "memory");
-    src = a.src[s_idx];
+    src = a.k.src[s_idx];
   }
   cs.img_ptr = src + ((size_t)n * a.cin_per_src + c_in_src) * ((size_t)a.H * a.pitch);
   cs.wgt_ptr = a.wpk + (size_t)chunk * C::W_USED;
@@ -212,7 +226,7 @@
 };
 
 template <int COUT, typename G>
-__device__ __forceinline__ void make_loader_plan(const ConvArgs& a, int lane, int y0, int x0, LoaderPlan<COUT, G>& pl) {
+__device__ __forceinline__ void make_loader_plan(const ConvView& a, int lane, int y0, int x0, LoaderPlan<COUT, G>& pl) {
   using C = ConvCfg<COUT, G>;
 #pragma unroll
   for (int p = 0; p < C::PIECES; ++p) {
@@ -233,7 +247,7 @@
 }
 
 template <int COUT, typename G>
-__device__ __forceinline__ void run_loader(const ConvArgs& a, float* smem, int lane, int n, int y0, int x0) {
+__device__ __forceinline__ void run_loader(const ConvView& a, float* smem, int lane, int n, int y0, int x0) {
   using C = ConvCfg<COUT, G>;
   if constexpr ((LARVA_DIAG & 256) != 0) return;
   LoaderPlan<COUT, G> pl;
@@ -261,7 +275,7 @@
 };
 
 template <int COUT, typename G>
-__device__ __forceinline__ void reg_load(const ConvArgs& a, const ChunkSrc& cs, int y0, int x0, int tid,
+__device__ __forceinline__ void reg_load(const ConvView& a, const ChunkSrc& cs, int y0, int x0, int tid,
                                          RegStaging<COUT, G>& st) {
   using C = ConvCfg<COUT, G>;
   const size_t plane = (size_t)a.H * a.pitch;
@@ -386,7 +400,7 @@
 }
 
 template <typename G>
-__device__ __forceinline__ void decode_tile(const ConvArgs& a, int vb, int& n, int& y0, int& x0) {
+__device__ __forceinline__ void decode_tile(const ConvView& a, int vb, int& n, int& y0, int& x0) {
   const int tile = xcd_remap(vb, a.nwg);
   const int t2 = div_by_magic(tile, a.magic_tx);
   const int tx = tile - t2 * a.tiles_x;
@@ -396,15 +410,15 @@
   y0 = ty * G::ROWS;
 }
 
-template <int COUT, typename G, bool VEC, int EPI, int NCT, int PG0, int NPG, bool PERSIST = false>
-__device__ __forceinline__ void run_role(const ConvArgs& a, float* smem, int ct0, int wave, int n, int y0, int x0, int tid) {
+template <int COUT, typename G, bool VEC, int EPI, int NCT, int PG0, int NPG, bool PERSIST = false, bool WPRE = false>
+__device__ __forceinline__ void run_role(const ConvView& a, float* smem, int ct0, int wave, int n, int y0, int x0, int tid) {
   using C = ConvCfg<COUT, G>;
   static_assert(!VEC || C::LOADER, "the 16-byte path runs with a loader wave (2 * PIECES <= 63 for every instantiated shape)");
   static_assert(!PERSIST || VEC, "persistent tiles: the loader-wave path");
   const int lane = tid & 63;
   const int lr = lane & 15, lq = lane >> 4;
-  float* const out_ptr = a.out;
-  struct { int H, W, pitch, plain; } k = {a.H, a.W, a.pitch, a.plain_stores};
+  float* const out_ptr = a.k.out;
+  struct { int H, W, pitch, plain; } k = {a.H, a.W, a.pitch, a.k.plain_stores};
   asm volatile("" : "+s"(k.H), "+s"(k.W), "+s"(k.pitch), "+s"(k.plain));
 
   constexpr bool kShuffleEpi = (EPI == kEpiShuffle || EPI == kEpiShuffleBase || EPI == kEpiShuffleL1);
@@ -441,9 +455,9 @@
         if constexpr (kShuffleEpi) {
           const int HH = 4 * a.H, WW = 4 * a.W;
           const size_t idx = (((size_t)n * C::CT + (ct0 + c)) * HH + (4 * y + lq)) * WW + 4 * x;
-          if (want(0)) aux[0][c][p] = *reinterpret_cast<const f32x4*>(a.base + idx);
+          if (want(0)) aux[0][c][p] = *reinterpret_cast<const f32x4*>(a.k.base + idx);
           if constexpr (EPI == kEpiShuffleL1) {
-            if (want(1)) aux[1][c][p] = *reinterpret_cast<const f32x4*>(a.truth + idx);
+            if (want(1)) aux[1][c][p] = *reinterpret_cast<const f32x4*>(a.k.truth + idx);
           }
         } else if constexpr (kPixMajor && (PERSIST || G::COLS == 16)) {
           const unsigned plane = (unsigned)a.H * (unsigned)a.pitch;
@@ -458,35 +472,35 @@
                                                      (int)(COUT * plane * 4u), 0x00020000);
           };
           if constexpr (EPI == kEpiMask) {
-            if (want(0)) aux[0][c][p] = __builtin_bit_cast(f32x4, __builtin_amdgcn_raw_buffer_load_b128(image(a.mask), lane_off, soff, 0));
+            if (want(0)) aux[0][c][p] = __builtin_bit_cast(f32x4, __builtin_amdgcn_raw_buffer_load_b128(image(a.k.mask), lane_off, soff, 0));
           }
           if constexpr (EPI == kEpiRes1 || EPI == kEpiRes2) {
-            if (want(0)) aux[0][c][p] = __builtin_bit_cast(f32x4, __builtin_amdgcn_raw_buffer_load_b128(image(a.res0), lane_off, soff, 0));
+            if (want(0)) aux[0][c][p] = __builtin_bit_cast(f32x4, __builtin_amdgcn_raw_buffer_load_b128(image(a.k.res0), lane_off, soff, 0));
           }
           if constexpr (EPI == kEpiRes2) {
-            if (want(1)) aux[1][c][p] = __builtin_bit_cast(f32x4, __builtin_amdgcn_raw_buffer_load_b128(image(a.res1), lane_off, soff, 0));
+            if (want(1)) aux[1][c][p] = __builtin_bit_cast(f32x4, __builtin_amdgcn_raw_buffer_load_b128(image(a.k.res1), lane_off, soff, 0));
           }
         } else if constexpr (kPixMajor) {
           const size_t plane = (size_t)a.H * a.pitch;
           const int xb = min(x0 + pcol * 16 + lq * 4, a.pitch - 4);
           const size_t idx = ((size_t)n * COUT + (ct0 + c) * 16 + lr) * plane + (size_t)y * a.pitch + xb;
           if constexpr (EPI == kEpiMask) {
-            if (want(0)) aux[0][c][p] = *reinterpret_cast<const f32x4*>(a.mask + idx);
+            if (want(0)) aux[0][c][p] = *reinterpret_cast<const f32x4*>(a.k.mask + idx);
           }
           if constexpr (EPI == kEpiRes1 || EPI == kEpiRes2) {
-            if (want(0)) aux[0][c][p] = *reinterpret_cast<const f32x4*>(a.res0 + idx);
+            if (want(0)) aux[0][c][p] = *reinterpret_cast<const f32x4*>(a.k.res0 + idx);
           }
           if constexpr (EPI == kEpiRes2) {
-            if (want(1)) aux[1][c][p] = *reinterpret_cast<const f32x4*>(a.res1 + idx);
+            if (want(1)) aux[1][c][p] = *reinterpret_cast<const f32x4*>(a.k.res1 + idx);
           }
         } else {
           const size_t plane = (size_t)a.H * a.pitch;
           const size_t idx0 = ((size_t)n * COUT + (ct0 + c) * 16 + lq * 4) * plane + (size_t)y * a.pitch + x;
 #pragma unroll
           for (int r = 0; r < 4; ++r) {
-            if constexpr (EPI == kEpiMask) aux[0][c][p][r] = a.mask[idx0 + r * plane];
-            if constexpr (EPI == kEpiRes1 || EPI == kEpiRes2) aux[0][c][p][r] = a.res0[idx0 + r * plane];
-            if constexpr (EPI == kEpiRes2) aux[1][c][p][r] = a.res1[idx0 + r * plane];
+            if constexpr (EPI == kEpiMask) aux[0][c][p][r] = a.k.mask[idx0 + r * plane];
+            if constexpr (EPI == kEpiRes1 || EPI == kEpiRes2) aux[0][c][p][r] = a.k.res0[idx0 + r * plane];
+            if constexpr (EPI == kEpiRes2) aux[1][c][p][r] = a.k.res1[idx0 + r * plane];
           }
         }
       }
@@ -541,7 +555,7 @@
       make_plan<COUT, G, true>(a, wave, lane, y0, x0, pl);
 #pragma unroll
       for (int i = 0; i < C::NPW; ++i)
-        if (wave + 4 * i >= C::IN_PIECES) dma_piece<COUT, G>(pl, i, wave, cs0, st0);
+        if (!WPRE && wave + 4 * i >= C::IN_PIECES) dma_piece<COUT, G>(pl, i, wave, cs0, st0);
       __builtin_amdgcn_sched_barrier(0);
       stamp(7);
       load_early();
@@ -606,7 +620,7 @@
   if constexpr (EPI == kEpiShuffleL1) {
     const int HH = 4 * k.H, WW = 4 * k.W;
     const size_t plane = (size_t)k.H * k.pitch;
-    const float g = a.gval;
+    const float g = a.k.gval;
     float s = 0.f;
 #pragma unroll
     for (int c = 0; c < NCT; ++c)
@@ -625,12 +639,12 @@
           const size_t idx0 = ((size_t)n * COUT + (ct0 + c) * 16 + lq * 4) * plane + (size_t)y * k.pitch + x;
 #pragma unroll
           for (int r = 0; r < 4; ++r)
-            __builtin_nontemporal_store(d[r] > 0.f ? g : (d[r] < 0.f ? -g : 0.f), &a.grad[idx0 + r * plane]);
+            __builtin_nontemporal_store(d[r] > 0.f ? g : (d[r] < 0.f ? -g : 0.f), &a.k.grad[idx0 + r * plane]);
         }
       }
 #pragma unroll
     for (int o = 32; o > 0; o >>= 1) s += __shfl_xor(s, o);
-    if (lane == 0) a.partial[4 * blockIdx.x + wave] = s;
+    if (lane == 0) a.k.partial[4 * blockIdx.x + wave] = s;
   } else if constexpr (EPI == kEpiShuffle || EPI == kEpiShuffleBase) {
     const int HH = 4 * k.H, WW = 4 * k.W;
 #pragma unroll
@@ -726,15 +740,30 @@
   }
 }
 
-__device__ __forceinline__ void fetch_args(const ConvArgs& a) {
-  asm volatile("" ::"s"(a.src[0]), "s"(a.wpk), "s"(a.bias), "s"(a.out), "s"(a.cin_per_src), "s"(a.n_chunks), "s"(a.N),
+struct ArgBatch {
+  const float* out;
+  const unsigned* tile_tab;
+  int N, plain_stores, tab_n, tab_lo, tab_hi;
+};
+__device__ __forceinline__ ArgBatch request_args(const ConvView& a) {
+  return ArgBatch{a.k.out, a.k.tile_tab, a.k.N, a.k.plain_stores, a.k.tab_n, a.k.tab16[0], a.k.tab16[16]};
+}
+__device__ __forceinline__ void fetch_args(const ConvView& a, const ArgBatch& b) {
+  asm volatile("" ::"s"(a.src0), "s"(a.wpk), "s"(a.bias), "s"(b.out), "s"(a.cin_per_src), "s"(a.n_chunks), "s"(b.N),
                "s"(a.H), "s"(a.W), "s"(a.pitch), "s"(a.tiles_x), "s"(a.tiles_y), "s"(a.magic_tx), "s"(a.magic_ty),
-               "s"(a.magic_cps), "s"(a.nwg), "s"(a.tile_tab), "s"(a.plain_stores), "s"(a.tab_n),
-               "s"(a.tab16[0]), "s"(a.tab16[16]));
-}
+               "s"(a.magic_cps), "s"(a.nwg), "s"(b.tile_tab), "s"(b.plain_stores), "s"(b.tab_n),
+               "s"(b.tab_lo), "s"(b.tab_hi));
+}
+__device__ __forceinline__ void fetch_args(const ConvView& a) { fetch_args(a, request_args(a)); }
+
+#define LARVA_TILE_PARAMS                                                                                             \
+  const float *wpk, const float *src0, unsigned long long magic_tx, unsigned long long magic_ty, int nwg, int tiles_x, \
+      int tiles_y, int H, int W, int pitch
+#define LARVA_TILE_VIEW(k) \
+  ConvView { wpk, src0, (k).bias, H, W, pitch, (k).cin_per_src, (k).n_chunks, nwg, tiles_x, tiles_y, magic_tx, magic_ty, (k).magic_cps, (k) }
 
 template <int COUT, bool VEC, int EPI, typename G = GeoWide>
-__device__ __forceinline__ void conv_tile(const ConvArgs& a, float* smem) {
+__device__ __forceinline__ void conv_tile(const ConvView& a, float* smem) {
   if constexpr ((LARVA_DIAG & 8) != 0) return;
   stamp(0);
   fetch_args(a);
@@ -776,20 +805,20 @@
 }
 
 template <int COUT, bool VEC, int EPI>
-__global__ __launch_bounds__(VEC ? ConvCfg<COUT>::THREADS_DMA : 256, VEC ? kWgPerCu : 1) void conv3x3_mfma_kernel(ConvArgs a) {
+__global__ __launch_bounds__(VEC ? ConvCfg<COUT>::THREADS_DMA : 256, VEC ? kWgPerCu : 1) void conv3x3_mfma_kernel(LARVA_TILE_PARAMS, ConvArgs k) {
   extern __shared__ __attribute__((aligned(16))) float smem[];
-  conv_tile<COUT, VEC, EPI>(a, smem);
+  conv_tile<COUT, VEC, EPI>(LARVA_TILE_VIEW(k), smem);
 }
 
 template <int COUT, int EPI>
-__global__ __launch_bounds__((ConvCfg<COUT, GeoWide4>::THREADS_DMA), kWgPerCu) void conv3x3_mfma_rows4_kernel(ConvArgs a) {
+__global__ __launch_bounds__((ConvCfg<COUT, GeoWide4>::THREADS_DMA), kWgPerCu) void conv3x3_mfma_rows4_kernel(LARVA_TILE_PARAMS, ConvArgs k) {
   extern __shared__ __attribute__((aligned(16))) float smem[];
-  conv_tile<COUT, true, EPI, GeoWide4>(a, smem);
+  conv_tile<COUT, true, EPI, GeoWide4>(LARVA_TILE_VIEW(k), smem);
 }
 static_assert(2 * ConvCfg<48, GeoWide4>::LDS_BYTES_DMA <= 160 * 1024, "two 4 x 48 workgroups per CU");
 
 template <int COUT, typename G>
-__device__ __forceinline__ void run_loader_persist(const ConvArgs& a, float* smem, int lane) {
+__device__ __forceinline__ void run_loader_persist(const ConvView& a, float* smem, int lane) {
   using C = ConvCfg<COUT, G>;
   static_assert(C::NST == 3 && 2 * C::PIECES <= 63, "three stages, two chunks in flight");
   LoaderPlan<COUT, G> pl;
@@ -835,9 +864,10 @@
 }
 
 template <int COUT, int EPI>
-__global__ __launch_bounds__((ConvCfg<COUT>::THREADS_DMA), kWgPerCu) void conv3x3_mfma_persist_kernel(ConvArgs a) {
+__global__ __launch_bounds__((ConvCfg<COUT>::THREADS_DMA), kWgPerCu) void conv3x3_mfma_persist_kernel(LARVA_TILE_PARAMS, ConvArgs k) {
   extern __shared__ __attribute__((aligned(16))) float smem[];
   using G = GeoWide;
+  const ConvView a = LARVA_TILE_VIEW(k);
   stamp(0);
   fetch_args(a);
   const int tid = threadIdx.x;
@@ -860,7 +890,7 @@
 }
 
 template <int COUT, int EPI, typename G>
-__device__ __forceinline__ void strip_roles(const ConvArgs& a, float* smem, int wave, int n, int y0, int x0, int tid) {
+__device__ __forceinline__ void strip_roles(const ConvView& a, float* smem, int wave, int n, int y0, int x0, int tid) {
   static_assert(ConvCfg<COUT, G>::LOADER, "the strip kernel is launched with a loader wave");
   static_assert(COUT == 48 || COUT == 32 || COUT == 64, "strip tiles: 32, 48 or 64 output channels");
   if (wave == 4) {
@@ -868,40 +898,62 @@
     return;
   }
   if constexpr (COUT == 64) {
-    run_role<COUT, G, true, EPI, 1, 0, G::ROWS>(a, smem, wave, wave, n, y0, x0, tid);
+    run_role<COUT, G, true, EPI, 1, 0, G::ROWS, false, true>(a, smem, wave, wave, n, y0, x0, tid);
   } else if constexpr (COUT == 48) {
-    if (wave < 3) run_role<COUT, G, true, EPI, 1, 0, G::ROWS - 1>(a, smem, wave, wave, n, y0, x0, tid);
-    else run_role<COUT, G, true, EPI, 3, G::ROWS - 1, 1>(a, smem, 0, wave, n, y0, x0, tid);
+    if (wave < 3) run_role<COUT, G, true, EPI, 1, 0, G::ROWS - 1, false, true>(a, smem, wave, wave, n, y0, x0, tid);
+    else run_role<COUT, G, true, EPI, 3, G::ROWS - 1, 1, false, true>(a, smem, 0, wave, n, y0, x0, tid);
   } else if constexpr (G::ROWS == 5) {
-    if (wave < 2) run_role<COUT, G, true, EPI, 1, 0, 3>(a, smem, wave, wave, n, y0, x0, tid);
-    else if (wave == 2) run_role<COUT, G, true, EPI, 2, 3, 1>(a, smem, 0, wave, n, y0, x0, tid);
-    else run_role<COUT, G, true, EPI, 2, 4, 1>(a, smem, 0, wave, n, y0, x0, tid);
+    if (wave < 2) run_role<COUT, G, true, EPI, 1, 0, 3, false, true>(a, smem, wave, wave, n, y0, x0, tid);
+    else if (wave == 2) run_role<COUT, G, true, EPI, 2, 3, 1, false, true>(a, smem, 0, wave, n, y0, x0, tid);
+    else run_role<COUT, G, true, EPI, 2, 4, 1, false, true>(a, smem, 0, wave, n, y0, x0, tid);
   } else {
-    if (wave < 2) run_role<COUT, G, true, EPI, 1, 0, 2>(a, smem, wave, wave, n, y0, x0, tid);
-    else run_role<COUT, G, true, EPI, 1, 2, 2>(a, smem, wave - 2, wave, n, y0, x0, tid);
+    if (wave < 2) run_role<COUT, G, true, EPI, 1, 0, 2, false, true>(a, smem, wave, wave, n, y0, x0, tid);
+    else run_role<COUT, G, true, EPI, 1, 2, 2, false, true>(a, smem, wave - 2, wave, n, y0, x0, tid);
   }
 }
 
 template <int COUT, int EPI>
-__global__ __launch_bounds__(320, kWgPerCu) void conv3x3_mfma_strip_kernel(ConvArgs a) {
+__global__ __launch_bounds__(320, kWgPerCu) void conv3x3_mfma_strip_kernel(
+    const float* wpk, const float* src0, const float* bias, unsigned long long magic_tx, int nwg, int tiles_x, int H, int W,
+    int pitch, int cin_per_src, ConvArgs k) {
   extern __shared__ __attribute__((aligned(16))) float smem[];
+  using C5 = ConvCfg<COUT, GeoS5>;
+  using C4 = ConvCfg<COUT, GeoS4>;
+  static_assert(C5::IN_PIECES == C4::IN_PIECES && C5::PIECES == C4::PIECES && C5::NPW == C4::NPW,
+                "both strip stages: the same pieces, dealt alike");
+  const ConvView a{wpk, src0, bias, H, W, pitch, cin_per_src, k.n_chunks, nwg, tiles_x, k.tiles_y, magic_tx, k.magic_ty, k.magic_cps, k};
   stamp(0);
-  fetch_args(a);
+  const int tid = threadIdx.x;
+  const int wave = __builtin_amdgcn_readfirstlane(tid >> 6);
+  __builtin_amdgcn_s_setprio(1);
   const int tile = xcd_remap(blockIdx.x, a.nwg);
   const int n = div_by_magic(tile, a.magic_tx);
   const int slot = tile - n * a.tiles_x;
+  const ArgBatch rest = request_args(a);
+  const int tab_n = rest.tab_n;
+  const unsigned pair = (unsigned)a.k.tab16[min(slot >> 1, 31)];
+  if constexpr (!(LARVA_DIAG & 2)) {
+    if (wave < 4) {
+      DmaPlan<COUT, GeoS5> pl;
+      make_plan<COUT, GeoS5, true>(a, wave, tid & 63, 0, 0, pl);
+      ChunkSrc cw;
+      cw.wgt_ptr = cw.img_ptr = a.wpk;
+      cw.wgt = cw.img = dma_rsrc(a.wpk);
+      const unsigned st0 = lds_addr_of(smem);
+#pragma unroll
+      for (int i = 0; i < C5::NPW; ++i)
+        if (wave + 4 * i >= C5::IN_PIECES) dma_piece<COUT, GeoS5>(pl, i, wave, cw, st0);
+    }
+  }
+  fetch_args(a, rest);
   unsigned e;
-  if (a.tab_n) {
-    const unsigned pair = (unsigned)a.tab16[slot >> 1];
+  if (tab_n) {
     const unsigned h = (slot & 1) ? pair >> 16 : pair & 0xffffu;
     e = (h & 0xffu) | (((h >> 8) & 0x7fu) << 16) | ((h >> 15) << 31);
   } else {
-    e = a.tile_tab[slot];
+    e = rest.tile_tab[slot];
   }
   const int y0 = (int)(e & 0xfffu), x0 = (int)((e >> 12) & 0xfffu);
-  const int tid = threadIdx.x;
-  const int wave = __builtin_amdgcn_readfirstlane(tid >> 6);
-  __builtin_amdgcn_s_setprio(1);
   if (e >> 31) strip_roles<COUT, EPI, GeoS5>(a, smem, wave, n, y0, x0, tid);
   else strip_roles<COUT, EPI, GeoS4>(a, smem, wave, n, y0, x0, tid);
 }
@@ -916,9 +968,14 @@
 };
 
 template <int COUT, int EPI>
-__global__ __launch_bounds__(ConvCfg<COUT>::THREADS_DMA, kWgPerCu) void conv3x3_mfma_batch_kernel(ConvBatch b) {
+__global__ __launch_bounds__(ConvCfg<COUT>::THREADS_DMA, kWgPerCu) void conv3x3_mfma_batch_kernel(
+    unsigned long long magic_tx, unsigned long long magic_ty, unsigned long long magic_cps, int nwg, int tiles_x, int tiles_y,
+    int H, int W, int pitch, int cin_per_src, int n_chunks, ConvBatch b) {
   extern __shared__ __attribute__((aligned(16))) float smem[];
-  conv_tile<COUT, true, EPI>(b.job[blockIdx.y], smem);
+  const ConvArgs& k = b.job[blockIdx.y];
+  conv_tile<COUT, true, EPI>(ConvView{k.wpk, k.src[0], k.bias, H, W, pitch, cin_per_src, n_chunks, nwg, tiles_x, tiles_y,
+                                      magic_tx, magic_ty, magic_cps, k},
+                             smem);
 }
 
 constexpr int kMaxPackJobs = 64;
@@ -1027,14 +1084,14 @@
   hipEvent_t start, stop;
 };
 
-template <auto Kernel, typename Args>
-static hipError_t launch(dim3 grid, dim3 block, size_t lds, hipStream_t stream, const LaunchTiming* tm, const Args& a) {
+template <auto Kernel, typename... Args>
+static hipError_t launch(dim3 grid, dim3 block, size_t lds, hipStream_t stream, const LaunchTiming* tm, const Args&... a) {
   static PerDeviceOnce lds_set;
   if (const hipError_t e = ensure_dynamic_lds(lds_set, reinterpret_cast<const void*>(Kernel), lds); e != hipSuccess) return e;
   if (tm)
-    hipExtLaunchKernelGGL(Kernel, grid, block, lds, stream, tm->start, tm->stop, 0, a);
+    hipExtLaunchKernelGGL(Kernel, grid, block, lds, stream, tm->start, tm->stop, 0, a...);
   else
-    hipLaunchKernelGGL(Kernel, grid, block, lds, stream, a);
+    hipLaunchKernelGGL(Kernel, grid, block, lds, stream, a...);
   return hipGetLastError();
 }
 
@@ -1067,6 +1124,8 @@
   }
 }
 
+#define LARVA_TILE_LEAD(a) (a).wpk, (a).src[0], (a).magic_tx, (a).magic_ty, (a).nwg, (a).tiles_x, (a).tiles_y, (a).H, (a).W, (a).pitch
+
 static int conv_slots() { return kWgPerCu * device_cu_count(); }
 
 template <int COUT>
@@ -1076,8 +1135,9 @@
   return with_epi(EpiAll{}, epi, hipErrorInvalidValue, [&](auto e) {
     constexpr int EPI = decltype(e)::value;
     if (vec)
-      return launch<conv3x3_mfma_kernel<COUT, true, EPI>>(grid, dim3(C::THREADS_DMA), C::LDS_BYTES_DMA, stream, tm, a);
-    return launch<conv3x3_mfma_kernel<COUT, false, EPI>>(grid, dim3(256), C::LDS_BYTES_REG, stream, tm, a);
+      return launch<conv3x3_mfma_kernel<COUT, true, EPI>>(grid, dim3(C::THREADS_DMA), C::LDS_BYTES_DMA, stream, tm,
+                                                          LARVA_TILE_LEAD(a), a);
+    return launch<conv3x3_mfma_kernel<COUT, false, EPI>>(grid, dim3(256), C::LDS_BYTES_REG, stream, tm, LARVA_TILE_LEAD(a), a);
   });
 }
 
@@ -1086,7 +1146,7 @@
   using C = ConvCfg<COUT, GeoWide4>;
   return with_epi(EpiRows4{}, epi, hipErrorNotSupported, [&](auto e) {
     return launch<conv3x3_mfma_rows4_kernel<COUT, decltype(e)::value>>(dim3(a.nwg), dim3(C::THREADS_DMA), C::LDS_BYTES_DMA,
-                                                                      stream, tm, a);
+                                                                      stream, tm, LARVA_TILE_LEAD(a), a);
   });
 }
 
@@ -1097,7 +1157,7 @@
   const int grid = a.nwg < conv_slots() ? a.nwg : conv_slots();
   return with_epi(EpiPersist{}, epi, hipErrorNotSupported, [&](auto e) {
     return launch<conv3x3_mfma_persist_kernel<COUT, decltype(e)::value>>(dim3(grid), dim3(C::THREADS_DMA), C::LDS_BYTES_DMA,
-                                                                        stream, tm, a);
+                                                                        stream, tm, LARVA_TILE_LEAD(a), a);
   });
 }
 
@@ -1109,7 +1169,9 @@
   return with_epi(Set{}, epi, epi == kEpiShuffleL1 ? hipErrorNotSupported : hipErrorInvalidValue, [&](auto e) {
     return launch<conv3x3_mfma_batch_kernel<COUT, decltype(e)::value>>(dim3(a.N * a.tiles_x * a.tiles_y, njobs),
                                                                       dim3(C::THREADS_DMA), C::LDS_BYTES_DMA, stream,
-                                                                      nullptr, b);
+                                                                      nullptr, a.magic_tx, a.magic_ty, a.magic_cps, a.nwg,
+                                                                      a.tiles_x, a.tiles_y, a.H, a.W, a.pitch, a.cin_per_src,
+                                                                      a.n_chunks, b);
   });
 }
 
@@ -1117,7 +1179,8 @@
 static hipError_t launch_strip(const ConvArgs& a, int epi, hipStream_t stream, const LaunchTiming* tm) {
   return with_epi(EpiAll{}, epi, hipErrorInvalidValue, [&](auto e) {
     return launch<conv3x3_mfma_strip_kernel<COUT, decltype(e)::value>>(dim3(a.nwg), dim3(320), kStripLdsBytes<COUT>, stream,
-                                                                      tm, a);
+                                                                      tm, a.wpk, a.src[0], a.bias, a.magic_tx, a.nwg, a.tiles_x,
+                                                                      a.H, a.W, a.pitch, a.cin_per_src, a);
   });
 }
 
```
